# ax-le/nn-fac

Measured on NVIDIA B200. Metric: NMF outer iters/sec (HALS & MU beta=1) at 65536x8192 r=64, higher is better.
Workload: dtype f32

## Files before the change

include/nnfac_b200.h:

```cpp
#ifndef NNFAC_B200_H
#define NNFAC_B200_H

#include <stddef.h>
#include <stdint.h>

#ifdef __cplusplus
extern "C" {
#endif

#define NNFAC_ABI_VERSION 1

typedef enum { NNFAC_F32 = 0, NNFAC_F64 = 1 } nnfac_dtype;

typedef enum {
  NNFAC_OK = 0,
  NNFAC_ERR_ARG = -1,
  NNFAC_ERR_CUDA = -2,
  NNFAC_ERR_UNSUPPORTED = -3,
  NNFAC_ERR_ALLOC = -4
} nnfac_status;

#define NNFAC_HALS_NORMALIZE 1u
#define NNFAC_HALS_NONZERO 2u
#define NNFAC_HALS_NO_TC 4u

typedef struct nnfac_ctx nnfac_ctx;

int nnfac_abi_version(void);
const char* nnfac_last_error(void);
int nnfac_ctx_create(int device, nnfac_ctx** out);
int nnfac_ctx_destroy(nnfac_ctx* ctx);
int nnfac_ctx_sm_count(const nnfac_ctx* ctx);
int64_t nnfac_ctx_launch_count(const nnfac_ctx* ctx);

int nnfac_ctx_board_export(nnfac_ctx* ctx, void* handle_out);
int nnfac_ctx_board_attach(nnfac_ctx* ctx, int world, int rank, const void* handles);
int nnfac_ctx_collective(nnfac_ctx* ctx, int on, const int64_t* slice_lengths);
int nnfac_ctx_sweep_variant(nnfac_ctx* ctx, int mode);

typedef struct nnfac_xchg nnfac_xchg;
int nnfac_xchg_create(nnfac_ctx* ctx, int64_t stage_floats, int64_t send_floats, nnfac_xchg** out);
int nnfac_xchg_export(nnfac_xchg* x, void* handle_out);
int nnfac_xchg_attach(nnfac_xchg* x, int world, int rank, const void* handles);
int nnfac_xchg_destroy(nnfac_xchg* x);
void* nnfac_xchg_ptr(nnfac_xchg* x, int which);
int nnfac_xchg_post(nnfac_xchg* x, int phase, void* stream);
int nnfac_xchg_post_tail(nnfac_xchg* x, const float* tail_src, int rows, int64_t pitch, int64_t col, void* stream);
int nnfac_xchg_pull_tail(nnfac_xchg* x, int which, float* out, int64_t ld_out, int r, int64_t pitch, int64_t col, int tail, void* stream);
int nnfac_xchg_inbox_mu_apply(nnfac_xchg* x, int64_t inbox_off, int nslabs, int64_t slab_stride, int64_t chunk, int64_t tail_pitch,
                              const float* F, int64_t ld_f, int r, int64_t lo, int64_t ncols, double floor_value, int64_t ld_send,
                              void* stream);

int nnfac_hals_nnls(nnfac_ctx* ctx, int dtype, const void* UtM, int64_t ld_utm, const void* UtU,
                    int64_t ld_utu, void* V, int64_t ld_v, int r, int64_t n, int maxiter,
                    double delta, double sparsity, unsigned flags, double* result, void* stream);
int nnfac_hals_solve_f32(nnfac_ctx* ctx, const float* UtM, int64_t ld_utm, const float* UtU, int64_t ld_utu,
                         const float* Vin, int64_t ld_vin, float* Vout, int64_t ld_vout, int r, int64_t n, int maxiter,
                         double delta, double sparsity, double* result, void* stream);
int nnfac_hals_solve_slabs_f32(nnfac_ctx* ctx, const float* UtM, int64_t ld_utm, int nslabs, int64_t slab_stride, int r_pad,
                               float* scratch, const float* UtU, int64_t ld_utu, const float* Vin, int64_t ld_vin, float* Vout,
                               int64_t ld_vout, int r, int64_t n, int maxiter, double delta, double sparsity, double* result,
                               void* stream);

int nnfac_gemm_strided(nnfac_ctx* ctx, int dtype, void* C, int64_t ldc, int64_t sc_b, const void* A,
                       int64_t sa_i, int64_t sa_k, int64_t sa_q, int64_t sa_b, const void* B,
                       int64_t sb_k, int64_t sb_j, int64_t sb_q, int64_t sb_b, int64_t M, int64_t N,
                       int64_t K, int64_t kb, int64_t batch, void* stream);

int nnfac_gram(nnfac_ctx* ctx, int dtype, void* out, int64_t ld_out, const void* F, int64_t ld_f, int r,
               int64_t len, void* stream);

int nnfac_mu_terms(nnfac_ctx* ctx, int dtype, double beta, const void* K, const void* X, void* P,
                   void* Q, int64_t count, void* stream);

int nnfac_mu_apply(nnfac_ctx* ctx, int dtype, void* F_out, const void* F_in, const void* num,
                   const void* den_mat, const void* den_vec, int vec_per_row, int64_t rows,
                   int64_t cols, double gamma, double floor_value, void* stream);

int nnfac_beta_divergence(nnfac_ctx* ctx, int dtype, double beta, const void* A, const void* B,
                          int64_t count, double* out, void* stream);

int nnfac_sq_diff(nnfac_ctx* ctx, int dtype, const void* A, const void* B, int64_t count,
                  double* out, void* stream);

int nnfac_dot(nnfac_ctx* ctx, int dtype, const void* A, const void* B, int64_t count, double* out,
              void* stream);

int nnfac_row_sums(nnfac_ctx* ctx, int dtype, const void* A, int64_t lda, int64_t rows,
                   int64_t cols, void* out, void* stream);

int nnfac_norm1(nnfac_ctx* ctx, int dtype, const void* A, int64_t lda, int64_t rows, int64_t cols,
                double* out, void* stream);

int nnfac_transpose(nnfac_ctx* ctx, int dtype, void* out, int64_t ld_out, const void* in,
                    int64_t ld_in, int64_t rows, int64_t cols, void* stream);

int nnfac_khatri_rao(nnfac_ctx* ctx, int dtype, void* out, const void* A, int64_t I, const void* B,
                     int64_t J, int64_t r, void* stream);

int nnfac_hadamard(nnfac_ctx* ctx, int dtype, void* out, const void* A, const void* B,
                   int64_t count, void* stream);
int nnfac_axpby(nnfac_ctx* ctx, int dtype, void* out, double a, const void* X, double b, const void* Y, int64_t count,
                void* stream);

int nnfac_core_pg_step(nnfac_ctx* ctx, int dtype, void* core, const void* MtX, const void* P, int64_t count, double step,
                       double sparse, double delta, double* state, void* stream);
int nnfac_core_pg_step_dev(nnfac_ctx* ctx, int dtype, void* core, const void* MtX, const void* P, int64_t count, double delta,
                           double* state, void* stream);
int nnfac_core_pg_step3(nnfac_ctx* ctx, int dtype, void* core, const void* MtX, const void* M0, const void* M1, const void* M2,
                        int r0, int r1, int r2, void* Z, double step, double sparse, int dev_scalars, double delta, double* state,
                        void* stream);
int nnfac_normalize_rows(nnfac_ctx* ctx, int dtype, void* A, int64_t lda, int64_t rows,
                         int64_t cols, void* stream);

typedef struct nnfac_nmf_plan nnfac_nmf_plan;
int nnfac_nmf_plan_create(nnfac_ctx* ctx, int64_t m, int64_t n, int r, nnfac_nmf_plan** out);
int nnfac_nmf_plan_bytes(nnfac_ctx* ctx, int64_t m, int64_t n, int r, size_t* bytes);
int nnfac_nmf_plan_create_in(nnfac_ctx* ctx, int64_t m, int64_t n, int r, void* workspace, size_t workspace_bytes,
                             void* stream, nnfac_nmf_plan** out);
int nnfac_nmf_plan_bytes_sided(nnfac_ctx* ctx, int64_t m, int64_t n, int r, int sides, size_t* bytes);
int nnfac_nmf_plan_create_sided(nnfac_ctx* ctx, int64_t m, int64_t n, int r, int sides, void* workspace, size_t workspace_bytes,
                                void* stream, nnfac_nmf_plan** out);
int nnfac_nmf_plan_bytes_planes(nnfac_ctx* ctx, int64_t m, int64_t n, int r, int sides, int planes, size_t* bytes);
int nnfac_nmf_plan_create_planes(nnfac_ctx* ctx, int64_t m, int64_t n, int r, int sides, int planes, void* workspace,
                                 size_t workspace_bytes, void* stream, nnfac_nmf_plan** out);
int nnfac_nmf_plan_view_bytes(nnfac_ctx* ctx, const nnfac_nmf_plan* base, int64_t left, int64_t I, int64_t right, int r, size_t* bytes);
int nnfac_nmf_plan_create_view(nnfac_ctx* ctx, const nnfac_nmf_plan* base, int64_t left, int64_t I, int64_t right, int r,
                               void* workspace, size_t workspace_bytes, void* stream, nnfac_nmf_plan** out);
int nnfac_nmf_plan_destroy(nnfac_nmf_plan* plan);
int nnfac_nmf_plan_load_x(nnfac_nmf_plan* plan, const float* X, int64_t ldx, void* stream);
int nnfac_nmf_plan_load_x_rows(nnfac_nmf_plan* plan, const float* Xrows, int64_t ldx, int64_t row0, int64_t rows, void* stream);
int nnfac_nmf_plan_load_x_done(nnfac_nmf_plan* plan, void* stream);
int nnfac_nmf_plan_f32_bytes(const nnfac_nmf_plan* plan, size_t* bytes);
int nnfac_nmf_plan_enable_f32(nnfac_nmf_plan* plan, void* workspace, size_t workspace_bytes, void* stream);
int nnfac_nmf_plan_cross(nnfac_nmf_plan* plan, int which, const float* F, int64_t ldf, float* out,
                         int64_t ld_out, void* stream);
int nnfac_nmf_plan_set_krao(nnfac_nmf_plan* plan, const float* At, int64_t lda, int64_t I, const float* Bt, int64_t ldb,
                            int64_t J, void* stream);
int nnfac_nmf_plan_set_krao_rows(nnfac_nmf_plan* plan, const float* At, int64_t lda, int64_t I, const float* Bt, int64_t ldb,
                                 int64_t J, void* stream);
int nnfac_nmf_plan_reduce(nnfac_nmf_plan* plan, int side, float* out, int64_t ld_out, void* stream);
int nnfac_nmf_plan_reduce_chunked(nnfac_nmf_plan* plan, int side, float* out, int64_t chunk, int slabs, const float* tail,
                                  int64_t ld_tail, int tail_cols, void* stream);
int nnfac_nmf_plan_set_factor(nnfac_nmf_plan* plan, int which, const float* Ft, int64_t ld, void* stream);
int nnfac_nmf_plan_set_factor_gathered(nnfac_nmf_plan* plan, int which, const float* G, int64_t chunk, float* Ft_out,
                                       int64_t ld_out, void* stream);
int nnfac_nmf_plan_set_factor_pulled(nnfac_nmf_plan* plan, int which, const nnfac_xchg* x, int64_t chunk, int64_t pitch,
                                     float* Ft_out, int64_t ld_out, void* stream);
int nnfac_nmf_plan_set_push(nnfac_nmf_plan* plan, const nnfac_xchg* x, int64_t inbox_off, int64_t chunk, int* slabs,
                            int64_t* slab_stride);
int nnfac_reduce_slabs_f32(nnfac_ctx* ctx, const float* slabs, int64_t ld, int nslabs, int r, int r_pad, int64_t n, float* out,
                           int64_t ld_out, void* stream);
int nnfac_nmf_plan_hals_solve(nnfac_nmf_plan* plan, int which, const float* UtM, int64_t ld_utm, const float* UtU,
                              int64_t ld_utu, const float* F_in, int64_t ld_in, float* F_out, int64_t ld_out, int maxiter,
                              double delta, double sparsity, double* result, void* stream);
int nnfac_nmf_plan_fused(nnfac_nmf_plan* plan, int side, int mode, int want_cost, float* out, int64_t ld_out,
                         double* cost_out, void* stream);
int nnfac_nmf_plan_mu_finish(nnfac_nmf_plan* plan, int which, const float* F_in, int64_t ld_in, const float* den,
                             double floor_value, float* F_out, int64_t ld_out, void* stream);
int nnfac_nmf_plan_fused_beta_bytes(const nnfac_nmf_plan* plan, size_t* bytes);
int nnfac_nmf_plan_fused_beta(nnfac_nmf_plan* plan, int side, double beta, int want_cost, float* den_partial, double* cost_out,
                              void* stream);
int nnfac_nmf_plan_mu_finish_beta(nnfac_nmf_plan* plan, int which, const float* F_in, int64_t ld_in, const float* den_partial,
                                  double gamma, double floor_value, float* F_out, int64_t ld_out, void* stream);
int nnfac_nmf_plan_info(const nnfac_nmf_plan* plan, int which, int* splits, int* stages_per_unit,
                        int* num_units, int* num_stages, int* grid);

int nnfac_philox_uniform(nnfac_ctx* ctx, float* out, int64_t ld, int64_t rows, int64_t cols, int64_t row0, int64_t col0,
                         uint64_t seed, uint32_t stream_id, double scale, int accumulate, void* stream);

#ifdef __cplusplus
}
#endif
#endif
```

nn-fac_b200/csrc/tc_common.cuh:

```cuda
#pragma once
#include <cuda.h>
#include <cuda_bf16.h>
#include <stdint.h>

namespace tc {

__device__ __forceinline__ uint32_t smem_u32(const void* p) {
  return (uint32_t)__cvta_generic_to_shared(p);
}

__device__ __forceinline__ void mbar_init(uint64_t* bar, uint32_t count) {
  asm volatile("mbarrier.init.shared::cta.b64 [%0], %1;" ::"r"(smem_u32(bar)), "r"(count) : "memory");
}
__device__ __forceinline__ void fence_barrier_init() {
  asm volatile("fence.mbarrier_init.release.cluster;" ::: "memory");
}
__device__ __forceinline__ void mbar_arrive_expect_tx(uint64_t* bar, uint32_t bytes) {
  asm volatile("mbarrier.arrive.expect_tx.shared::cta.b64 _, [%0], %1;" ::"r"(smem_u32(bar)), "r"(bytes) : "memory");
}
__device__ __forceinline__ void mbar_arrive(uint64_t* bar) {
  asm volatile("mbarrier.arrive.shared::cta.b64 _, [%0];" ::"r"(smem_u32(bar)) : "memory");
}
__device__ __forceinline__ bool mbar_try_wait(uint64_t* bar, uint32_t parity) {
  uint32_t ok;
  asm volatile(
      "{\n"
      " .reg .pred p;\n"
      " mbarrier.try_wait.parity.shared::cta.b64 p, [%1], %2;\n"
      " selp.u32 %0, 1, 0, p;\n"
      "}\n"
      : "=r"(ok)
      : "r"(smem_u32(bar)), "r"(parity)
      : "memory");
  return ok != 0;
}
__device__ __forceinline__ uint64_t global_ns() {
  uint64_t t;
  asm volatile("mov.u64 %0, %globaltimer;" : "=l"(t));
  return t;
}
static __device__ __noinline__ void mbar_wait_timeout_check(uint64_t& t0) {
  const uint64_t now = global_ns();
  if (t0 == 0) t0 = now;
  else if (now - t0 > 4000000000ull) __trap();
}
__device__ __forceinline__ void mbar_wait(uint64_t* bar, uint32_t parity) {
  if (mbar_try_wait(bar, parity)) return;
  uint64_t t0 = 0;
  for (;;) {
#pragma unroll 1
    for (uint32_t spins = 0; spins < 4096u; ++spins)
      if (mbar_try_wait(bar, parity)) return;
    mbar_wait_timeout_check(t0);
  }
}

__device__ __forceinline__ void fence_proxy_async_smem() {
  asm volatile("fence.proxy.async.shared::cta;" ::: "memory");
}
__device__ __forceinline__ void tcgen05_fence_before() {
  asm volatile("tcgen05.fence::before_thread_sync;" ::: "memory");
}
__device__ __forceinline__ void tcgen05_fence_after() {
  asm volatile("tcgen05.fence::after_thread_sync;" ::: "memory");
}

__device__ __forceinline__ void prefetch_tmap(const CUtensorMap* m) {
  asm volatile("prefetch.tensormap [%0];" ::"l"(reinterpret_cast<uint64_t>(m)) : "memory");
}
__device__ __forceinline__ void tma_load_2d(void* smem_dst, const CUtensorMap* m, uint64_t* bar, int c0, int c1) {
  asm volatile(
      "cp.async.bulk.tensor.2d.shared::cluster.global.tile.mbarrier::complete_tx::bytes [%0], [%1, {%3, %4}], [%2];"
      ::"r"(smem_u32(smem_dst)), "l"(reinterpret_cast<uint64_t>(m)), "r"(smem_u32(bar)), "r"(c0), "r"(c1)
      : "memory");
}
__device__ __forceinline__ void tma_load_2d_hint(void* smem_dst, const CUtensorMap* m, uint64_t* bar, int c0, int c1,
                                                 uint64_t policy) {
  asm volatile(
      "cp.async.bulk.tensor.2d.shared::cluster.global.tile.mbarrier::complete_tx::bytes.L2::cache_hint [%0], [%1, {%3, %4}], [%2], %5;"
      ::"r"(smem_u32(smem_dst)), "l"(reinterpret_cast<uint64_t>(m)), "r"(smem_u32(bar)), "r"(c0), "r"(c1), "l"(policy)
      : "memory");
}
__device__ __forceinline__ void tma_load_3d_hint(void* smem_dst, const CUtensorMap* m, uint64_t* bar, int c0, int c1, int c2,
                                                 uint64_t policy) {
  asm volatile(
      "cp.async.bulk.tensor.3d.shared::cluster.global.tile.mbarrier::complete_tx::bytes.L2::cache_hint [%0], [%1, {%3, %4, %5}], [%2], %6;"
      ::"r"(smem_u32(smem_dst)), "l"(reinterpret_cast<uint64_t>(m)), "r"(smem_u32(bar)), "r"(c0), "r"(c1), "r"(c2), "l"(policy)
      : "memory");
}
constexpr uint64_t kEvictFirst = 0x12F0000000000000ull;
constexpr uint64_t kEvictLast = 0x14F0000000000000ull;

__device__ __forceinline__ void tmem_alloc(uint32_t* smem_result, uint32_t ncols) {
  asm volatile("tcgen05.alloc.cta_group::1.sync.aligned.shared::cta.b32 [%0], %1;" ::"r"(smem_u32(smem_result)), "r"(ncols)
               : "memory");
  asm volatile("tcgen05.relinquish_alloc_permit.cta_group::1.sync.aligned;" ::: "memory");
}
__device__ __forceinline__ void tmem_dealloc(uint32_t taddr, uint32_t ncols) {
  asm volatile("tcgen05.dealloc.cta_group::1.sync.aligned.b32 %0, %1;" ::"r"(taddr), "r"(ncols) : "memory");
}
__device__ __forceinline__ void tmem_ld16(uint32_t taddr, uint32_t (&v)[16]) {
  asm volatile(
      "tcgen05.ld.sync.aligned.32x32b.x16.b32 {%0,%1,%2,%3,%4,%5,%6,%7,%8,%9,%10,%11,%12,%13,%14,%15}, [%16];"
      : "=r"(v[0]), "=r"(v[1]), "=r"(v[2]), "=r"(v[3]), "=r"(v[4]), "=r"(v[5]), "=r"(v[6]), "=r"(v[7]), "=r"(v[8]),
        "=r"(v[9]), "=r"(v[10]), "=r"(v[11]), "=r"(v[12]), "=r"(v[13]), "=r"(v[14]), "=r"(v[15])
      : "r"(taddr)
      : "memory");
}
__device__ __forceinline__ void tmem_ld32(uint32_t taddr, uint32_t (&v)[32]) {
  asm volatile(
      "tcgen05.ld.sync.aligned.32x32b.x32.b32 {%0,%1,%2,%3,%4,%5,%6,%7,%8,%9,%10,%11,%12,%13,%14,%15,"
      "%16,%17,%18,%19,%20,%21,%22,%23,%24,%25,%26,%27,%28,%29,%30,%31}, [%32];"
      : "=r"(v[0]), "=r"(v[1]), "=r"(v[2]), "=r"(v[3]), "=r"(v[4]), "=r"(v[5]), "=r"(v[6]), "=r"(v[7]), "=r"(v[8]),
        "=r"(v[9]), "=r"(v[10]), "=r"(v[11]), "=r"(v[12]), "=r"(v[13]), "=r"(v[14]), "=r"(v[15]), "=r"(v[16]),
        "=r"(v[17]), "=r"(v[18]), "=r"(v[19]), "=r"(v[20]), "=r"(v[21]), "=r"(v[22]), "=r"(v[23]), "=r"(v[24]),
        "=r"(v[25]), "=r"(v[26]), "=r"(v[27]), "=r"(v[28]), "=r"(v[29]), "=r"(v[30]), "=r"(v[31])
      : "r"(taddr)
      : "memory");
}
__device__ __forceinline__ void tmem_st16(uint32_t taddr, const uint32_t (&v)[16]) {
  asm volatile(
      "tcgen05.st.sync.aligned.32x32b.x16.b32 [%0], {%1,%2,%3,%4,%5,%6,%7,%8,%9,%10,%11,%12,%13,%14,%15,%16};"
      ::"r"(taddr), "r"(v[0]), "r"(v[1]), "r"(v[2]), "r"(v[3]), "r"(v[4]), "r"(v[5]), "r"(v[6]), "r"(v[7]), "r"(v[8]),
        "r"(v[9]), "r"(v[10]), "r"(v[11]), "r"(v[12]), "r"(v[13]), "r"(v[14]), "r"(v[15])
      : "memory");
}
__device__ __forceinline__ void tmem_st8(uint32_t taddr, const uint32_t (&v)[8]) {
  asm volatile("tcgen05.st.sync.aligned.32x32b.x8.b32 [%0], {%1,%2,%3,%4,%5,%6,%7,%8};"
               ::"r"(taddr), "r"(v[0]), "r"(v[1]), "r"(v[2]), "r"(v[3]), "r"(v[4]), "r"(v[5]), "r"(v[6]), "r"(v[7])
               : "memory");
}
__device__ __forceinline__ void tmem_ld_wait16(uint32_t (&v)[16]) {
  asm volatile("tcgen05.wait::ld.sync.aligned;"
               : "+r"(v[0]), "+r"(v[1]), "+r"(v[2]), "+r"(v[3]), "+r"(v[4]), "+r"(v[5]), "+r"(v[6]), "+r"(v[7]), "+r"(v[8]),
                 "+r"(v[9]), "+r"(v[10]), "+r"(v[11]), "+r"(v[12]), "+r"(v[13]), "+r"(v[14]), "+r"(v[15])
               :
               : "memory");
}
__device__ __forceinline__ void tmem_st_wait() { asm volatile("tcgen05.wait::st.sync.aligned;" ::: "memory"); }
__device__ __forceinline__ void tmem_ld_wait() { asm volatile("tcgen05.wait::ld.sync.aligned;" ::: "memory"); }

__device__ __forceinline__ uint64_t umma_desc_k_sw128(uint32_t smem_addr) {
  uint64_t d = 0;
  d |= (uint64_t)((smem_addr >> 4) & 0x3FFF);
  d |= (uint64_t)1 << 16;
  d |= (uint64_t)(1024 >> 4) << 32;
  d |= (uint64_t)1 << 46;
  d |= (uint64_t)2 << 61;
  return d;
}
__device__ __forceinline__ uint64_t umma_desc_mn_sw128(uint32_t smem_addr) {
  uint64_t d = 0;
  d |= (uint64_t)((smem_addr >> 4) & 0x3FFF);
  d |= (uint64_t)(8192 >> 4) << 16;
  d |= (uint64_t)(1024 >> 4) << 32;
  d |= (uint64_t)1 << 46;
  d |= (uint64_t)2 << 61;
  return d;
}
__device__ __forceinline__ uint32_t umma_idesc_bf16(int M, int N) {
  return (1u << 4) | (1u << 7) | (1u << 10) | ((uint32_t)(N >> 3) << 17) | ((uint32_t)(M >> 4) << 24);
}
__device__ __forceinline__ void umma_bf16(uint32_t tmem_d, uint64_t adesc, uint64_t bdesc, uint32_t idesc, bool accumulate) {
  asm volatile(
      "{\n"
      " .reg .pred p;\n"
      " setp.ne.b32 p, %4, 0;\n"
      " tcgen05.mma.cta_group::1.kind::f16 [%0], %1, %2, %3, p;\n"
      "}\n" ::"r"(tmem_d), "l"(adesc), "l"(bdesc), "r"(idesc), "r"((uint32_t)accumulate)
      : "memory");
}
__device__ __forceinline__ void umma_bf16_ts(uint32_t tmem_d, uint32_t tmem_a, uint64_t bdesc, uint32_t idesc, bool accumulate) {
  asm volatile(
      "{\n"
      " .reg .pred p;\n"
      " setp.ne.b32 p, %4, 0;\n"
      " tcgen05.mma.cta_group::1.kind::f16 [%0], [%1], %2, %3, p;\n"
      "}\n" ::"r"(tmem_d), "r"(tmem_a), "l"(bdesc), "r"(idesc), "r"((uint32_t)accumulate)
      : "memory");
}
__device__ __forceinline__ void umma_commit(uint64_t* bar) {
  asm volatile("tcgen05.commit.cta_group::1.mbarrier::arrive::one.shared::cluster.b64 [%0];" ::"r"(smem_u32(bar)) : "memory");
}

__device__ __forceinline__ bool elect_one() {
  uint32_t pred;
  asm volatile(
      "{\n"
      " .reg .pred p;\n"
      " elect.sync _|p, 0xffffffff;\n"
      " selp.u32 %0, 1, 0, p;\n"
      "}\n"
      : "=r"(pred));
  return pred != 0;
}

__device__ __forceinline__ void split_bf16(float x, __nv_bfloat16& hi, __nv_bfloat16& lo) {
  hi = __float2bfloat16_rn(x);
  lo = __float2bfloat16_rn(x - __bfloat162float(hi));
}

__device__ __forceinline__ void split3_bf16(float x, __nv_bfloat16& hi, __nv_bfloat16& mid, __nv_bfloat16& lo) {
  hi = __float2bfloat16_rn(x);
  if (isinf(__bfloat162float(hi)) && isfinite(x)) hi = __float2bfloat16_rz(x);
  const float r = x - __bfloat162float(hi);
  mid = __float2bfloat16_rn(r);
  lo = __float2bfloat16_rn(r - __bfloat162float(mid));
}

}
```

nn-fac_b200/csrc/tc_fused.cu:

```cuda
#include "tc_plan.cuh"

#include <string.h>

namespace {
using namespace tcplan;

constexpr int NSP = 4;
constexpr int CW = 64 / NSP;
constexpr int NCHK = CW / 8;
constexpr int NWT = 4 * NSP;
constexpr int FUSED_THREADS = 128 + 32 * NWT;
static_assert(CW == 16, "the transform below moves 16 columns per tcgen05.ld / 8 words per tcgen05.st");
constexpr uint32_t X_BYTES = TILE_ROWS * BK * sizeof(bf16);
constexpr int MODE_RES = 0, MODE_MU = 1, MODE_BETA0 = 2, MODE_BETAI = 3, MODE_BETAG = 4;
#ifndef FUSED_PREFETCH
#define FUSED_PREFETCH 0
#endif
#ifndef FUSED_PACKED
#define FUSED_PACKED 1
#endif
#ifndef FUSED_DEFER_COST
#define FUSED_DEFER_COST 1
#endif
constexpr int DRAIN = 2;

template <int RK, int PLANES = 2, bool XF32 = false>
struct Cfg {
  static constexpr int KR = RK / 64;
  static constexpr uint32_t FK_BYTES = (uint32_t)KR * 64 * BK * sizeof(bf16);
  static constexpr uint32_t XB = (PLANES == 3 && !XF32 ? 3 : 2) * X_BYTES;
  static constexpr uint32_t STAGE_BYTES = XB + PLANES * FK_BYTES;
  static constexpr int FSTAGES = PLANES == 3 ? (XF32 ? 3 : 2) : RK == 64 ? 4 : 3;
  static constexpr int ND1 = PLANES == 3 && XF32 ? 2 : RK == 64 ? 3 : 2;
  static constexpr uint32_t A1_BYTES = RK == 64 ? PLANES * X_BYTES : 0;
  static constexpr int CWD = RK / NSP;
  static constexpr size_t SMEM = A1_BYTES + (size_t)FSTAGES * STAGE_BYTES + 512;
};

struct FusedParams {
  int r_pad, splits, stages_per_unit, num_units, drain, want_cost, tiles, split_major;
  int64_t ld_partial;
  float* partial;
  double* cost_part;
  const bf16 *a1h, *a1l;
  int64_t R;
  float* push[NNFAC_MAX_PEERS];
  int64_t push_chunk;
  int push_src;
};

constexpr int NHC = 11;
struct BetaParams {
  float* den;
  float beta, bm2;
  int ibm2, ibeta;
  float inv_bb1, inv_beta;
  float hc[NHC];
};

__device__ __forceinline__ float rcp_approx(float x) {
  float y;
  asm("rcp.approx.ftz.f32 %0, %1;" : "=f"(y) : "f"(x));
  return y;
}
__device__ __forceinline__ float lg2_approx(float x) {
  float y;
  asm("lg2.approx.ftz.f32 %0, %1;" : "=f"(y) : "f"(x));
  return y;
}
__device__ __forceinline__ float kl_g(float q) {
  const float d = q - 1.f;
  if (fabsf(d) < 0.0625f) {
    float c = fmaf(d, -1.f / 42.f, 1.f / 30.f);
    c = fmaf(d, c, -1.f / 20.f);
    c = fmaf(d, c, 1.f / 12.f);
    c = fmaf(d, c, -1.f / 6.f);
    c = fmaf(d, c, 0.5f);
    return d * d * c;
  }
  return fmaf(q, lg2_approx(q + 1e-30f) * 0.6931471805599453f, -d);
}
__device__ __forceinline__ float ex2_approx(float x) {
  float y;
  asm("ex2.approx.ftz.f32 %0, %1;" : "=f"(y) : "f"(x));
  return y;
}
__device__ __forceinline__ float ipow(float b, int n) {
  float r = 1.f;
  for (; n; n >>= 1, b *= b)
    if (n & 1) r *= b;
  return r;
}
template <int MODE>
__device__ __forceinline__ float beta_cost(float x, float k, float kb, float ik, const BetaParams& bp) {
  if (!(k > 0.f)) return 0.f;
  if (x == 0.f) return MODE == MODE_BETA0 ? -1.f : kb * bp.inv_beta;
  const float q = x * ik, d = q - 1.f;
  float h;
  if (fabsf(d) < 0.25f) {
    float c = bp.hc[NHC - 1];
#pragma unroll
    for (int i = NHC - 2; i >= 0; --i) c = fmaf(d, c, bp.hc[i]);
    h = d * d * c;
  } else if (MODE == MODE_BETA0) {
    h = fmaf(lg2_approx(q), -0.6931471805599453f, d);
  } else {
    const float qb = MODE == MODE_BETAI ? ipow(q, bp.ibeta) : ex2_approx(bp.beta * lg2_approx(q));
    h = (fmaf(-bp.beta, q, qb) + (bp.beta - 1.f)) * bp.inv_bb1;
  }
  return kb * h;
}
__device__ __forceinline__ float bf_lo(uint32_t w) { return __uint_as_float(w << 16); }
__device__ __forceinline__ float bf_hi(uint32_t w) { return __uint_as_float(w & 0xffff0000u); }

template <int MODE, bool COST, bool XF32, int RK, int PLANES = 2>
__global__ void __launch_bounds__(FUSED_THREADS, 1)
tc_fused_kernel(const __grid_constant__ CUtensorMap map_xh, const __grid_constant__ CUtensorMap map_xl,
                const __grid_constant__ CUtensorMap map_fkh, const __grid_constant__ CUtensorMap map_fkl,
                const __grid_constant__ CUtensorMap map_a1h, const __grid_constant__ CUtensorMap map_a1l,
                const FusedParams p, const __grid_constant__ CUtensorMap map_xm, const __grid_constant__ CUtensorMap map_fkm,
                const __grid_constant__ CUtensorMap map_a1m, const BetaParams bp) {
  using C = Cfg<RK, PLANES, PLANES == 3 && XF32>;
  constexpr bool BETA = MODE >= MODE_BETA0;
  static_assert(!BETA || (RK == 64 && PLANES == 2), "general beta: 2 planes, rank <= 64");
  static_assert(RK == 64 || (MODE == MODE_RES && !XF32), "rank 65..128: residual + cross-product pass only");
  static_assert(PLANES == 2 || (RK == 64 && (MODE == MODE_RES) != XF32), "3 planes: rank <= 64; beta = 1 reads X from its fp32 copy");
  constexpr int FSTAGES = C::FSTAGES, ND1 = BETA ? 2 : C::ND1, CWD = C::CWD;
  constexpr int NQ = BETA ? 1 : 2;
  constexpr int DRAIN_P = PLANES == 3 ? 1 : DRAIN;
  constexpr uint32_t FK_BYTES = C::FK_BYTES, STAGE_BYTES = C::STAGE_BYTES, A1_BYTES = C::A1_BYTES, XB = C::XB;
  extern __shared__ __align__(1024) uint8_t smem[];
  uint8_t* a1 = smem;
  uint8_t* ring = smem + A1_BYTES;
  uint64_t* bars = reinterpret_cast<uint64_t*>(ring + (size_t)FSTAGES * STAGE_BYTES);
  uint64_t* full = bars;
  uint64_t* empty = bars + 4;
  uint64_t* a1_full = bars + 9;
  uint64_t* a1_empty = bars + 10;
  uint64_t* d1_full = bars + 11;
  uint64_t* d1_empty = bars + 14;
  uint64_t* d2_full = bars + 17;
  uint64_t* d2_empty = bars + 19;
  uint64_t* a1t_ready = bars + 21;
  uint64_t* a1t_free = bars + 22;
  uint64_t* q_ready = bars + 23;
  uint64_t* q_free = bars + 25;
  uint32_t* tmem_slot = reinterpret_cast<uint32_t*>(bars + 27);
  double* cost_sh = reinterpret_cast<double*>(bars + 28);

  const int warp = threadIdx.x >> 5, lane = threadIdx.x & 31;

  if (warp == 0 && lane == 0) {
    tc::prefetch_tmap(&map_xh); tc::prefetch_tmap(&map_xl);
    tc::prefetch_tmap(&map_fkh); tc::prefetch_tmap(&map_fkl);
    if (RK == 64) { tc::prefetch_tmap(&map_a1h); tc::prefetch_tmap(&map_a1l); }
    if (PLANES == 3) { if (!XF32) tc::prefetch_tmap(&map_xm); tc::prefetch_tmap(&map_fkm); tc::prefetch_tmap(&map_a1m); }
  }
  if (warp == 1 && lane == 0) {
    for (int s = 0; s < FSTAGES; ++s) { tc::mbar_init(&full[s], 1); tc::mbar_init(&empty[s], NWT + 1); }
    tc::mbar_init(a1_full, 1); tc::mbar_init(a1_empty, BETA ? 1 : NWT);
    tc::mbar_init(a1t_ready, NWT); tc::mbar_init(a1t_free, 1);
    for (int b = 0; b < 2; ++b) { tc::mbar_init(&q_ready[b], NWT); tc::mbar_init(&q_free[b], 1); }
    for (int b = 0; b < ND1; ++b) { tc::mbar_init(&d1_full[b], 1); tc::mbar_init(&d1_empty[b], NWT); }
    for (int b = 0; b < 2; ++b) { tc::mbar_init(&d2_full[b], 1); tc::mbar_init(&d2_empty[b], NWT); }
    tc::fence_barrier_init();
  }
  if (warp == 2) tc::tmem_alloc(tmem_slot, 512);
  tc::tcgen05_fence_before();
  __syncthreads();
  tc::tcgen05_fence_after();
  const uint32_t tmem_base = *tmem_slot;
  const uint32_t D1 = tmem_base, D2 = tmem_base + 64 * ND1, A1T = D2 + 2 * RK, QT = BETA ? A1T + 2 * RK : A1T + PLANES * (RK / 2);
  const uint32_t D2D = A1T;
  const int S = p.stages_per_unit;

  if (warp == 0 && lane == 0) {
    int stage = 0; uint32_t phase = 0, a1_phase = 0;
    for (int u = blockIdx.x; u < p.num_units; u += gridDim.x) {
      const int tile = p.split_major ? u % p.tiles : u / p.splits, split = p.split_major ? u / p.tiles : u % p.splits;
      const int row0 = tile * TILE_ROWS, k0 = split * S * BK;
      if (RK == 64) {
        tc::mbar_wait(a1_empty, a1_phase ^ 1);
        a1_phase ^= 1;
        tc::mbar_arrive_expect_tx(a1_full, A1_BYTES);
        tc::tma_load_2d_hint(a1, &map_a1h, a1_full, 0, row0, tc::kEvictLast);
        tc::tma_load_2d_hint(a1 + X_BYTES, &map_a1l, a1_full, 0, row0, tc::kEvictLast);
        if (PLANES == 3) tc::tma_load_2d_hint(a1 + 2 * X_BYTES, &map_a1m, a1_full, 0, row0, tc::kEvictLast);
      }
      for (int ks = 0; ks < S; ++ks) {
        tc::mbar_wait(&empty[stage], phase ^ 1);
        uint8_t* st = ring + (size_t)stage * STAGE_BYTES;
        tc::mbar_arrive_expect_tx(&full[stage], STAGE_BYTES);
        const int c = k0 + ks * BK;
        tc::tma_load_2d_hint(st, &map_xh, &full[stage], c, row0, tc::kEvictFirst);
        tc::tma_load_2d_hint(st + X_BYTES, XF32 ? &map_xh : &map_xl, &full[stage], XF32 ? c + 32 : c, row0, tc::kEvictFirst);
        if (PLANES == 3 && !XF32) tc::tma_load_2d_hint(st + 2 * X_BYTES, &map_xm, &full[stage], c, row0, tc::kEvictFirst);
#pragma unroll
        for (int kr = 0; kr < C::KR; ++kr) {
          tc::tma_load_2d_hint(st + XB + kr * 8192, &map_fkh, &full[stage], kr * 64, c, tc::kEvictLast);
          tc::tma_load_2d_hint(st + XB + FK_BYTES + kr * 8192, &map_fkl, &full[stage], kr * 64, c, tc::kEvictLast);
          if (PLANES == 3) tc::tma_load_2d_hint(st + XB + 2 * FK_BYTES + kr * 8192, &map_fkm, &full[stage], kr * 64, c, tc::kEvictLast);
        }
        if (++stage == FSTAGES) { stage = 0; phase ^= 1; }
      }
    }
  } else if (warp == 1) {
    const uint32_t idesc1 = tc::umma_idesc_bf16(TILE_ROWS, 64);
    const int ksteps = p.r_pad / UMMA_K;
    int st1 = 0; uint32_t ph1 = 0;
    int b1 = 0; uint32_t b1_phase = 0;
    uint32_t a1_phase = 0;
    for (int u = blockIdx.x; u < p.num_units; u += gridDim.x) {
      tc::mbar_wait(BETA ? a1_full : a1t_ready, a1_phase);
      a1_phase ^= 1;
      for (int i = 0; i < S; ++i) {
        tc::mbar_wait(&full[st1], ph1);
        tc::mbar_wait(&d1_empty[b1], b1_phase ^ 1);
        tc::tcgen05_fence_after();
        if (tc::elect_one()) {
          const uint32_t sb = tc::smem_u32(ring + (size_t)st1 * STAGE_BYTES);
          const uint64_t fkh = tc::umma_desc_k_sw128(sb + XB), fkl = tc::umma_desc_k_sw128(sb + XB + FK_BYTES);
          const uint32_t d = D1 + (uint32_t)b1 * 64;
          if constexpr (PLANES == 3) {
            const uint64_t fkm = tc::umma_desc_k_sw128(sb + XB + 2 * FK_BYTES);
            const uint32_t ah = A1T, al = A1T + RK / 2, am = A1T + RK;
#pragma unroll
            for (int k = 0; k < RK / UMMA_K; ++k) {
              if (k < ksteps) {
                const uint64_t bo = (uint64_t)((k & 3) * 2);
                tc::umma_bf16_ts(d, al + 8 * k, fkh + bo, idesc1, k != 0);
                tc::umma_bf16_ts(d, am + 8 * k, fkm + bo, idesc1, true);
                tc::umma_bf16_ts(d, ah + 8 * k, fkl + bo, idesc1, true);
                tc::umma_bf16_ts(d, am + 8 * k, fkh + bo, idesc1, true);
                tc::umma_bf16_ts(d, ah + 8 * k, fkm + bo, idesc1, true);
              }
            }
#pragma unroll
            for (int k = 0; k < RK / UMMA_K; ++k)
              if (k < ksteps) tc::umma_bf16_ts(d, ah + 8 * k, fkh + (uint64_t)((k & 3) * 2), idesc1, true);
          } else if constexpr (BETA) {
            const uint64_t ah = tc::umma_desc_k_sw128(tc::smem_u32(a1)), al = tc::umma_desc_k_sw128(tc::smem_u32(a1 + X_BYTES));
#pragma unroll
            for (int k = 0; k < RK / UMMA_K; ++k) {
              if (k < ksteps) {
                const uint64_t ko = (uint64_t)(k * 2), bo = (uint64_t)((k & 3) * 2);
                tc::umma_bf16(d, ah + ko, fkh + bo, idesc1, k != 0);
                tc::umma_bf16(d, al + ko, fkh + bo, idesc1, true);
                tc::umma_bf16(d, ah + ko, fkl + bo, idesc1, true);
              }
            }
          } else {
#pragma unroll
          for (int k = 0; k < RK / UMMA_K; ++k) {
            if (k < ksteps) {
              const uint64_t bo = (uint64_t)((k >> 2) * (8192 >> 4) + (k & 3) * 2);
              tc::umma_bf16_ts(d, A1T + 8 * k, fkh + bo, idesc1, k != 0);
              tc::umma_bf16_ts(d, A1T + RK / 2 + 8 * k, fkh + bo, idesc1, true);
              tc::umma_bf16_ts(d, A1T + 8 * k, fkl + bo, idesc1, true);
            }
          }
          }
          tc::umma_commit(&d1_full[b1]);
          if (i == S - 1) tc::umma_commit(BETA ? a1_empty : a1t_free);
        }
        __syncwarp();
        if (++b1 == ND1) { b1 = 0; b1_phase ^= 1; }
        if (++st1 == FSTAGES) { st1 = 0; ph1 ^= 1; }
      }
    }
  } else if (warp == 3) {
    const uint32_t idesc2 = tc::umma_idesc_bf16(TILE_ROWS, p.r_pad) | (1u << 16);
    int qb = 0; uint32_t qb_phase = 0;
    int st2 = 0; uint32_t ph2 = 0;
    int b2 = 0; uint32_t b2_phase = 0;
    for (int u = blockIdx.x; u < p.num_units; u += gridDim.x) {
      for (int j = 0; j < S; ++j) {
        const bool chain_start = (j % DRAIN_P) == 0;
        const bool chain_end = ((j + 1) % DRAIN_P) == 0 || j == S - 1;
        tc::mbar_wait(&full[st2], ph2);
        if (MODE == MODE_MU || BETA) tc::mbar_wait(&q_ready[qb], qb_phase);
        if (chain_start) tc::mbar_wait(&d2_empty[b2], b2_phase ^ 1);
        tc::tcgen05_fence_after();
        if (tc::elect_one()) {
          const uint32_t sb = tc::smem_u32(ring + (size_t)st2 * STAGE_BYTES);
          const uint64_t xh = tc::umma_desc_k_sw128(sb), xl = tc::umma_desc_k_sw128(sb + X_BYTES);
          const uint64_t fnh = tc::umma_desc_mn_sw128(sb + XB);
          const uint64_t fnl = tc::umma_desc_mn_sw128(sb + XB + FK_BYTES);
          const uint32_t d = D2 + (uint32_t)b2 * RK;
          if constexpr (PLANES == 3) {
            const uint64_t fnm = tc::umma_desc_mn_sw128(sb + XB + 2 * FK_BYTES);
            const uint64_t xm = tc::umma_desc_k_sw128(sb + 2 * X_BYTES);
#pragma unroll
            for (int k = 0; k < BK / UMMA_K; ++k) {
              const uint64_t ko = (uint64_t)(k * 2), kb = (uint64_t)(k * 128);
              const bool acc0 = !(chain_start && k == 0);
              if (MODE == MODE_MU) {
                const uint32_t qa = QT + (uint32_t)qb * 64 + 8 * k;
                tc::umma_bf16_ts(d, qa, fnl + kb, idesc2, acc0);
                tc::umma_bf16_ts(d, qa + 32, fnm + kb, idesc2, true);
                tc::umma_bf16_ts(d, qa, fnm + kb, idesc2, true);
                tc::umma_bf16_ts(d, qa + 32, fnh + kb, idesc2, true);
              } else {
                tc::umma_bf16(d, xl + ko, fnh + kb, idesc2, acc0);
                tc::umma_bf16(d, xm + ko, fnm + kb, idesc2, true);
                tc::umma_bf16(d, xh + ko, fnl + kb, idesc2, true);
                tc::umma_bf16(d, xm + ko, fnh + kb, idesc2, true);
                tc::umma_bf16(d, xh + ko, fnm + kb, idesc2, true);
              }
            }
#pragma unroll
            for (int k = 0; k < BK / UMMA_K; ++k) {
              if (MODE == MODE_MU) tc::umma_bf16_ts(d, QT + (uint32_t)qb * 64 + 8 * k, fnh + (uint64_t)(k * 128), idesc2, true);
              else tc::umma_bf16(d, xh + (uint64_t)(k * 2), fnh + (uint64_t)(k * 128), idesc2, true);
            }
          } else if constexpr (BETA) {
            const uint32_t dd = D2D + (uint32_t)b2 * RK;
#pragma unroll
            for (int k = 0; k < BK / UMMA_K; ++k) {
              const uint64_t kb = (uint64_t)(k * 128);
              const uint32_t qa = QT + 8 * k, qd = qa + 64;
              const bool acc0 = !(chain_start && k == 0);
              tc::umma_bf16_ts(d, qa, fnh + kb, idesc2, acc0);
              tc::umma_bf16_ts(d, qa + 32, fnh + kb, idesc2, true);
              tc::umma_bf16_ts(d, qa, fnl + kb, idesc2, true);
              tc::umma_bf16_ts(dd, qd, fnh + kb, idesc2, acc0);
              tc::umma_bf16_ts(dd, qd + 32, fnh + kb, idesc2, true);
              tc::umma_bf16_ts(dd, qd, fnl + kb, idesc2, true);
            }
          } else {
#pragma unroll
          for (int k = 0; k < BK / UMMA_K; ++k) {
            const uint64_t ko = (uint64_t)(k * 2);
            const uint64_t kb = (uint64_t)(k * 128);
            if (MODE == MODE_MU) {
              const uint32_t qa = QT + (uint32_t)qb * 64 + 8 * k;
              tc::umma_bf16_ts(d, qa, fnh + kb, idesc2, !(chain_start && k == 0));
              tc::umma_bf16_ts(d, qa + 32, fnh + kb, idesc2, true);
              tc::umma_bf16_ts(d, qa, fnl + kb, idesc2, true);
            } else {
              tc::umma_bf16(d, xh + ko, fnh + kb, idesc2, !(chain_start && k == 0));
              tc::umma_bf16(d, xl + ko, fnh + kb, idesc2, true);
              tc::umma_bf16(d, xh + ko, fnl + kb, idesc2, true);
            }
          }
          }
          tc::umma_commit(&empty[st2]);
          if (MODE == MODE_MU || BETA) tc::umma_commit(&q_free[qb]);
          if (chain_end) tc::umma_commit(&d2_full[b2]);
        }
        __syncwarp();
        if (MODE == MODE_MU || BETA) { if (++qb == NQ) { qb = 0; qb_phase ^= 1; } }
        if (chain_end) { if (++b2 == 2) { b2 = 0; b2_phase ^= 1; } }
        if (++st2 == FSTAGES) { st2 = 0; ph2 ^= 1; }
      }
    }
  } else if (warp >= 4) {
    const int q = warp & 3, part = (warp - 4) >> 2;
    const int row = q * 32 + lane;
    const uint32_t lane_base = (uint32_t)(q * 32) << 16;
    int st = 0; uint32_t ph = 0;
    int b1 = 0; uint32_t b1_phase = 0;
    int b2 = 0; uint32_t b2_phase = 0;
    int qb = 0; uint32_t qb_phase = 0;
    uint32_t a1_phase = 0;
    double cost = 0.0, costk = 0.0;
    for (int u = blockIdx.x; u < p.num_units; u += gridDim.x) {
      const int tile = p.split_major ? u % p.tiles : u / p.splits, split = p.split_major ? u / p.tiles : u % p.splits;
      float sum[CWD], sumd[BETA ? CWD : 1];
#pragma unroll
      for (int j = 0; j < CWD; ++j) sum[j] = 0.f;
      if (BETA) {
#pragma unroll
        for (int j = 0; j < CWD; ++j) sumd[BETA ? j : 0] = 0.f;
      } else if (RK == 64) {
        tc::mbar_wait(a1_full, a1_phase);
        tc::mbar_wait(a1t_free, a1_phase ^ 1);
        a1_phase ^= 1;
        tc::tcgen05_fence_after();
#pragma unroll
        for (int pl = 0; pl < PLANES; ++pl) {
          uint32_t w[4 * NCHK];
#pragma unroll
          for (int cc = 0; cc < NCHK; ++cc) {
            const int chunk = NCHK * part + cc;
            const uint4 v4 = *reinterpret_cast<const uint4*>(a1 + pl * X_BYTES + (uint32_t)row * 128u + (uint32_t)((chunk ^ (row & 7)) << 4));
            w[4 * cc] = v4.x; w[4 * cc + 1] = v4.y; w[4 * cc + 2] = v4.z; w[4 * cc + 3] = v4.w;
          }
          tc::tmem_st8(A1T + lane_base + 32 * pl + (CW / 2) * part, w);
        }
        tc::tmem_st_wait();
        tc::tcgen05_fence_before();
        __syncwarp();
        if (lane == 0) { tc::mbar_arrive(a1t_ready); tc::mbar_arrive(a1_empty); }
      } else {
        const int64_t grow = (int64_t)tile * TILE_ROWS + row;
        uint32_t w[2][16];
#pragma unroll
        for (int pl = 0; pl < 2; ++pl) {
          const uint4* src = reinterpret_cast<const uint4*>((pl ? p.a1l : p.a1h) + grow * RK + part * (RK / 4));
#pragma unroll
          for (int c = 0; c < 4; ++c) {
            const uint4 v4 = grow < p.R ? __ldg(src + c) : make_uint4(0u, 0u, 0u, 0u);
            w[pl][4 * c] = v4.x; w[pl][4 * c + 1] = v4.y; w[pl][4 * c + 2] = v4.z; w[pl][4 * c + 3] = v4.w;
          }
        }
        tc::mbar_wait(a1t_free, a1_phase ^ 1);
        a1_phase ^= 1;
        tc::tcgen05_fence_after();
        tc::tmem_st16(A1T + lane_base + (RK / 8) * part, w[0]);
        tc::tmem_st16(A1T + lane_base + RK / 2 + (RK / 8) * part, w[1]);
        tc::tmem_st_wait();
        tc::tcgen05_fence_before();
        __syncwarp();
        if (lane == 0) tc::mbar_arrive(a1t_ready);
      }
      auto drain_chain = [&]() {
        tc::mbar_wait(&d2_full[b2], b2_phase);
        tc::tcgen05_fence_after();
#pragma unroll
        for (int c0 = 0; c0 < CWD; c0 += 16) {
          if (CWD * part + c0 < p.r_pad) {
            uint32_t v[16];
            tc::tmem_ld16(D2 + (uint32_t)b2 * RK + lane_base + CWD * part + c0, v);
            tc::tmem_ld_wait();
#pragma unroll
            for (int j = 0; j < 16; ++j) sum[c0 + j] += __uint_as_float(v[j]);
            if (BETA) {
              tc::tmem_ld16(D2D + (uint32_t)b2 * RK + lane_base + CWD * part + c0, v);
              tc::tmem_ld_wait();
#pragma unroll
              for (int j = 0; j < 16; ++j) sumd[BETA ? c0 + j : 0] += __uint_as_float(v[j]);
            }
          }
        }
        tc::tcgen05_fence_before();
        __syncwarp();
        if (lane == 0) tc::mbar_arrive(&d2_empty[b2]);
        if (++b2 == 2) { b2 = 0; b2_phase ^= 1; }
      };
      int drained = 0;
      float2 acc2 = make_float2(0.f, 0.f), acck2 = make_float2(0.f, 0.f);
      const float2 neg1 = make_float2(-1.f, -1.f), tiny2 = make_float2(1e-30f, 1e-30f);
      uint32_t kn[CW];
      int bf = b1; uint32_t bf_phase = b1_phase;
      auto fetch_d1 = [&]() {
        tc::mbar_wait(&d1_full[bf], bf_phase);
        tc::tcgen05_fence_after();
        tc::tmem_ld16(D1 + (uint32_t)bf * 64 + lane_base + CW * part, kn);
        if (++bf == ND1) { bf = 0; bf_phase ^= 1; }
      };
#if FUSED_PREFETCH
      fetch_d1();
#endif
      for (int i = 0; i < S; ++i) {
#if !FUSED_PREFETCH
        fetch_d1();
#endif
        tc::tmem_ld_wait16(kn);
        uint32_t kk[CW];
#pragma unroll
        for (int j = 0; j < CW; ++j) kk[j] = kn[j];
        tc::tcgen05_fence_before();
        __syncwarp();
        if (lane == 0) tc::mbar_arrive(&d1_empty[b1]);
        if (++b1 == ND1) { b1 = 0; b1_phase ^= 1; }
#if FUSED_PREFETCH
        if (i + 1 < S) fetch_d1();
#endif
        tc::mbar_wait(&full[st], ph);
        uint8_t* xh = ring + (size_t)st * STAGE_BYTES;
        uint8_t* xl = xh + X_BYTES;
        uint32_t qhw[4 * NCHK], qlw[4 * NCHK];
        constexpr bool DEFER = FUSED_DEFER_COST && FUSED_PACKED && MODE == MODE_MU && COST;
        float2 xs[DEFER ? 4 * NCHK : 1], qs[DEFER ? 4 * NCHK : 1];
        uint32_t dhw[BETA ? 4 * NCHK : 1], dlw[BETA ? 4 * NCHK : 1];
#pragma unroll
        for (int cc = 0; cc < NCHK; ++cc) {
          float2 xv[4];
          if (XF32) {
            const uint8_t* xb = xh + (size_t)(part >> 1) * X_BYTES + (uint32_t)row * 128u;
#pragma unroll
            for (int h = 0; h < 2; ++h) {
              const int chunk = 4 * (part & 1) + 2 * cc + h;
              const float4 v4 = *reinterpret_cast<const float4*>(xb + ((chunk ^ (row & 7)) << 4));
              xv[2 * h] = make_float2(v4.x, v4.y); xv[2 * h + 1] = make_float2(v4.z, v4.w);
            }
          } else {
            const int chunk = NCHK * part + cc;
            const uint32_t off = (uint32_t)row * 128u + (uint32_t)((chunk ^ (row & 7)) << 4);
            const uint4 h4 = *reinterpret_cast<const uint4*>(xh + off);
            const uint4 l4 = *reinterpret_cast<const uint4*>(xl + off);
            const uint32_t hw[4] = {h4.x, h4.y, h4.z, h4.w}, lw[4] = {l4.x, l4.y, l4.z, l4.w};
            if constexpr (PLANES == 3) {
              const uint4 m4 = *reinterpret_cast<const uint4*>(xl + X_BYTES + off);
              const uint32_t mw[4] = {m4.x, m4.y, m4.z, m4.w};
#pragma unroll
              for (int w = 0; w < 4; ++w)
                xv[w] = __fadd2_rn(make_float2(bf_lo(hw[w]), bf_hi(hw[w])),
                                   __fadd2_rn(make_float2(bf_lo(mw[w]), bf_hi(mw[w])), make_float2(bf_lo(lw[w]), bf_hi(lw[w]))));
            } else {
#pragma unroll
            for (int w = 0; w < 4; ++w)
#if FUSED_PACKED
              xv[w] = __fadd2_rn(make_float2(bf_lo(hw[w]), bf_hi(hw[w])), make_float2(bf_lo(lw[w]), bf_hi(lw[w])));
#else
              xv[w] = make_float2(bf_lo(hw[w]) + bf_lo(lw[w]), bf_hi(hw[w]) + bf_hi(lw[w]));
#endif
            }
          }
          if constexpr (BETA) {
#pragma unroll
            for (int w = 0; w < 4; ++w) {
              float an[2], ad[2];
#pragma unroll
              for (int h = 0; h < 2; ++h) {
                const float x = h ? xv[w].y : xv[w].x, k = __uint_as_float(kk[cc * 8 + 2 * w + h]);
                float ik = 0.f, pk, kb = 1.f;
                if (MODE == MODE_BETA0) {
                  ik = rcp_approx(k);
                  pk = ik * ik;
                  ad[h] = ik;
                } else {
                  pk = MODE == MODE_BETAI ? ipow(k, bp.ibm2) : ex2_approx(bp.bm2 * lg2_approx(k));
                  ad[h] = pk * k;
                  if (COST) { ik = rcp_approx(k); kb = ad[h] * k; }
                }
                an[h] = x * pk;
                if (!(k > 0.f)) { an[h] = 0.f; ad[h] = 0.f; }
                if (COST) acc2.x += beta_cost<MODE>(x, k, kb, ik, bp);
              }
              const __nv_bfloat162 hn = __floats2bfloat162_rn(an[0], an[1]), hd = __floats2bfloat162_rn(ad[0], ad[1]);
              const uint32_t hnw = *reinterpret_cast<const uint32_t*>(&hn), hdw = *reinterpret_cast<const uint32_t*>(&hd);
              const __nv_bfloat162 ln = __floats2bfloat162_rn(an[0] - bf_lo(hnw), an[1] - bf_hi(hnw));
              const __nv_bfloat162 ld = __floats2bfloat162_rn(ad[0] - bf_lo(hdw), ad[1] - bf_hi(hdw));
              qhw[4 * cc + w] = hnw;
              qlw[4 * cc + w] = *reinterpret_cast<const uint32_t*>(&ln);
              dhw[BETA ? 4 * cc + w : 0] = hdw;
              dlw[BETA ? 4 * cc + w : 0] = *reinterpret_cast<const uint32_t*>(&ld);
            }
          } else {
#if FUSED_PACKED
#pragma unroll
          for (int w = 0; w < 4; ++w) {
            const float2 x2 = xv[w];
            const float2 k2 = make_float2(__uint_as_float(kk[cc * 8 + 2 * w]), __uint_as_float(kk[cc * 8 + 2 * w + 1]));
            if (MODE == MODE_RES) {
              const float2 r2 = __ffma2_rn(k2, neg1, x2);
              acc2 = __ffma2_rn(r2, r2, acc2);
            } else {
              const float2 kt = __fadd2_rn(k2, tiny2);
              const float2 q2 = __fmul2_rn(x2, make_float2(rcp_approx(kt.x), rcp_approx(kt.y)));
              if (COST) {
                if (DEFER) {
                  xs[DEFER ? 4 * cc + w : 0] = x2; qs[DEFER ? 4 * cc + w : 0] = q2;
                } else {
                  const float2 qt = __fadd2_rn(q2, tiny2);
                  acc2 = __ffma2_rn(x2, make_float2(lg2_approx(qt.x), lg2_approx(qt.y)), acc2);
                }
                acck2 = __fadd2_rn(acck2, k2);
              }
              const __nv_bfloat162 hq = __floats2bfloat162_rn(q2.x, q2.y);
              const uint32_t hqw = *reinterpret_cast<const uint32_t*>(&hq);
              const float2 rem = __ffma2_rn(make_float2(bf_lo(hqw), bf_hi(hqw)), neg1, q2);
              const __nv_bfloat162 lq = __floats2bfloat162_rn(rem.x, rem.y);
              qhw[4 * cc + w] = hqw;
              qlw[4 * cc + w] = *reinterpret_cast<const uint32_t*>(&lq);
            }
          }
#else
#pragma unroll
          for (int w = 0; w < 4; ++w) {
            const float x0 = xv[w].x, x1 = xv[w].y;
            const float k0 = __uint_as_float(kk[cc * 8 + 2 * w]), k1 = __uint_as_float(kk[cc * 8 + 2 * w + 1]);
            if (MODE == MODE_RES) {
              const float r0 = x0 - k0, r1 = x1 - k1;
              acc2.x = fmaf(r0, r0, acc2.x);
              acc2.y = fmaf(r1, r1, acc2.y);
            } else {
              const float i0 = rcp_approx(fmaxf(k0, 1e-30f)), i1 = rcp_approx(fmaxf(k1, 1e-30f));
              const float q0 = x0 * i0, q1 = x1 * i1;
              if (COST) {
                acc2.x = fmaf(x0, lg2_approx(fmaxf(q0, 1e-30f)), acc2.x);
                acc2.y = fmaf(x1, lg2_approx(fmaxf(q1, 1e-30f)), acc2.y);
                acck2.x += k0; acck2.y += k1;
              }
              const __nv_bfloat162 hq = __floats2bfloat162_rn(q0, q1);
              const uint32_t hqw = *reinterpret_cast<const uint32_t*>(&hq);
              const __nv_bfloat162 lq = __floats2bfloat162_rn(q0 - bf_lo(hqw), q1 - bf_hi(hqw));
              qhw[4 * cc + w] = hqw;
              qlw[4 * cc + w] = *reinterpret_cast<const uint32_t*>(&lq);
            }
          }
#endif
          }
        }
        auto flush_cost = [&]() {
          if (COST && ((i & 7) == 7 || i == S - 1)) {
            cost += (double)(acc2.x + acc2.y);
            acc2 = make_float2(0.f, 0.f);
            if (MODE == MODE_MU) { costk += (double)(acck2.x + acck2.y); acck2 = make_float2(0.f, 0.f); }
          }
        };
        if (!DEFER) flush_cost();
        __syncwarp();
        if (lane == 0) tc::mbar_arrive(&empty[st]);
        if (++st == FSTAGES) { st = 0; ph ^= 1; }
        if (MODE == MODE_MU) {
          tc::mbar_wait(&q_free[qb], qb_phase ^ 1);
          tc::tcgen05_fence_after();
          const uint32_t qa = QT + (uint32_t)qb * 64 + lane_base + (CW / 2) * part;
          tc::tmem_st8(qa, qhw);
          tc::tmem_st8(qa + 32, qlw);
          tc::tmem_st_wait();
          tc::tcgen05_fence_before();
          __syncwarp();
          if (lane == 0) tc::mbar_arrive(&q_ready[qb]);
          if (++qb == NQ) { qb = 0; qb_phase ^= 1; }
          if (DEFER) {
#pragma unroll
            for (int e = 0; e < 4 * NCHK; ++e) {
              if constexpr (PLANES == 3) {
                const float2 k2 = make_float2(__uint_as_float(kk[2 * e]), __uint_as_float(kk[2 * e + 1]));
                acc2 = __ffma2_rn(k2, make_float2(kl_g(qs[DEFER ? e : 0].x), kl_g(qs[DEFER ? e : 0].y)), acc2);
              } else {
                const float2 qt = __fadd2_rn(qs[DEFER ? e : 0], tiny2);
                acc2 = __ffma2_rn(xs[DEFER ? e : 0], make_float2(lg2_approx(qt.x), lg2_approx(qt.y)), acc2);
              }
            }
            flush_cost();
          }
        }
        if constexpr (BETA) {
          tc::mbar_wait(&q_free[0], qb_phase ^ 1);
          tc::tcgen05_fence_after();
          const uint32_t qa = QT + lane_base + (CW / 2) * part;
          tc::tmem_st8(qa, qhw);
          tc::tmem_st8(qa + 32, qlw);
          tc::tmem_st8(qa + 64, dhw);
          tc::tmem_st8(qa + 96, dlw);
          tc::tmem_st_wait();
          tc::tcgen05_fence_before();
          __syncwarp();
          if (lane == 0) tc::mbar_arrive(&q_ready[0]);
          qb_phase ^= 1;
        }
        if (DRAIN_P == 2 ? (i >= 3 && (i & 1)) : i >= 2) { drain_chain(); ++drained; }
      }
      for (; drained < (S + DRAIN_P - 1) / DRAIN_P; ++drained) drain_chain();
      if (p.push_chunk > 0) {
        const int64_t row0 = (int64_t)tile * TILE_ROWS;
        const int q = (int)(row0 / p.push_chunk);
        float* out = p.push[q] + (((int64_t)p.push_src * p.splits + split) * p.r_pad + CWD * part) * p.push_chunk + (row0 - q * p.push_chunk) + row;
#pragma unroll
        for (int j = 0; j < CWD; ++j)
          if (CWD * part + j < p.r_pad) out[(int64_t)j * p.push_chunk] = sum[j];
      } else {
        float* out = p.partial + ((int64_t)split * p.r_pad + CWD * part) * p.ld_partial + (int64_t)tile * TILE_ROWS + row;
#pragma unroll
        for (int j = 0; j < CWD; ++j)
          if (CWD * part + j < p.r_pad) out[(int64_t)j * p.ld_partial] = sum[j];
        if (BETA) {
          float* outd = bp.den + ((int64_t)split * p.r_pad + CWD * part) * p.ld_partial + (int64_t)tile * TILE_ROWS + row;
#pragma unroll
          for (int j = 0; j < CWD; ++j)
            if (CWD * part + j < p.r_pad) outd[(int64_t)j * p.ld_partial] = sumd[BETA ? j : 0];
        }
      }
    }
    if (COST) {
      cost = warp_sum(cost);
      if (MODE == MODE_MU) costk = warp_sum(costk);
      if (lane == 0) { cost_sh[warp - 4] = cost; cost_sh[NWT + warp - 4] = costk; }
      asm volatile("bar.sync 1, %0;" ::"n"(32 * NWT) : "memory");
      if (warp == 4 && lane == 0) {
        double t = 0.0, tk = 0.0;
        for (int w = 0; w < NWT; ++w) { t += cost_sh[w]; tk += cost_sh[NWT + w]; }
        p.cost_part[blockIdx.x] = t;
        p.cost_part[512 + blockIdx.x] = tk;
      }
    }
  }
  tc::tcgen05_fence_before();
  __syncthreads();
  if (warp == 2) tc::tmem_dealloc(tmem_base, 512);
}

struct PeerG {
  const float* p[NNFAC_MAX_PEERS];
  const unsigned long long* flags;
  int world;
  unsigned long long seq;
};

template <bool APPLY, int RK, bool PULL, int PLANES = 2, bool DENP = false>
__global__ void __launch_bounds__(256) factor_finish_kernel(const float* __restrict__ partial, int splits, int r, int r_pad, int64_t R,
                                                            int64_t ldp, const float* __restrict__ F_in, int64_t ld_in,
                                                            int64_t in_chunk, int64_t in_slab, const PeerG G,
                                                            const float* __restrict__ den, float floor_value, float* __restrict__ F_out,
                                                            int64_t ld_out, bf16* __restrict__ fh, bf16* __restrict__ fl, int64_t ld_plane,
                                                            bf16* __restrict__ rowh, bf16* __restrict__ rowl,
                                                            bf16* __restrict__ fm = nullptr, bf16* __restrict__ rowm = nullptr,
                                                            float gamma = 1.f) {
  __shared__ float tile[RK][33];
  const int tx = threadIdx.x & 31, ty = threadIdx.x >> 5;
  if (PULL && G.flags != nullptr) {
    if ((int)threadIdx.x < G.world) {
      const unsigned long long* f = G.flags + NNFAC_MAX_PEERS + threadIdx.x;
      unsigned long long v, spins = 0;
      do {
        asm volatile("ld.acquire.sys.global.u64 %0, [%1];" : "=l"(v) : "l"(f) : "memory");
        if (++spins > (1ull << 27)) __trap();
      } while (v < G.seq);
    }
    __syncthreads();
  }
  const int64_t c0 = (int64_t)blockIdx.x * 32, c = c0 + tx;
  const int64_t cin = in_chunk > 0 ? (c / in_chunk) * in_slab + (c % in_chunk) : c;
  float pulled[PULL ? RK / 8 : 1];
  if (PULL) {
    const float* src = c < R ? G.p[c / in_chunk] + (c % in_chunk) : nullptr;
#pragma unroll
    for (int i = 0; i < RK / 8; ++i) {
      const int k = ty + 8 * i;
      pulled[i] = (k < r && c < R) ? __ldcv(src + (int64_t)k * ld_in) : 0.f;
    }
  }
#pragma unroll
  for (int k = ty; k < RK; k += 8) {
    float f = 0.f;
    if (k < r && c < R) {
      f = PULL ? pulled[PULL ? (k - ty) / 8 : 0] : F_in[(int64_t)k * ld_in + cin];
      if (APPLY) {
        auto sum_splits = [&](const float* __restrict__ part) {
          float s = 0.f;
          int sp = 0;
          for (; sp + 8 <= splits; sp += 8) {
            float t[8];
#pragma unroll
            for (int u = 0; u < 8; ++u) t[u] = part[((int64_t)(sp + u) * r_pad + k) * ldp + c];
#pragma unroll
            for (int u = 0; u < 8; ++u) s += t[u];
          }
          for (; sp < splits; ++sp) s += part[((int64_t)sp * r_pad + k) * ldp + c];
          return s;
        };
        const float num = sum_splits(partial);
        float v;
        if constexpr (DENP) {
          float ratio = num / sum_splits(den);
          if (gamma == 0.5f) ratio = sqrtf(ratio);
          else if (gamma != 1.f) ratio = powf(ratio, gamma);
          v = f * ratio;
        } else {
          v = f * (num / den[k]);
        }
        f = v > floor_value ? v : floor_value;
        if (v != v) f = v;
      }
      if (F_out) F_out[(int64_t)k * ld_out + c] = f;
      bf16 h, l;
      if constexpr (PLANES == 3) {
        bf16 md;
        tc::split3_bf16(f, h, md, l);
        fm[(int64_t)k * ld_plane + c] = md;
      } else {
        tc::split_bf16(f, h, l);
      }
      fh[(int64_t)k * ld_plane + c] = h;
      fl[(int64_t)k * ld_plane + c] = l;
    }
    tile[k][tx] = f;
  }
  if (rowh == nullptr) return;
  __syncthreads();
  for (int i = ty; i < 32; i += 8) {
    const int64_t cc = c0 + i;
    if (cc < R) {
#pragma unroll
      for (int h2 = 0; h2 < RK / 32; ++h2) {
        const int k = tx + 32 * h2;
        bf16 h, l;
        if constexpr (PLANES == 3) {
          bf16 md;
          tc::split3_bf16(tile[k][i], h, md, l);
          rowm[cc * RK + k] = md;
        } else {
          tc::split_bf16(tile[k][i], h, l);
        }
        rowh[cc * RK + k] = h;
        rowl[cc * RK + k] = l;
      }
    }
  }
}

__global__ void sum_cost_parts_kernel(const double* part, int n, double* out) {
  if (threadIdx.x == 0) {
    double s = 0.0;
    for (int i = 0; i < n; ++i) s += part[i];
    out[0] = s;
  }
}

__global__ void kl_cost_finish_kernel(const double* part, int n, const double* sums, double* out) {
  if (threadIdx.x == 0) {
    double s = 0.0, sk = 0.0;
    for (int i = 0; i < n; ++i) { s += part[i]; sk += part[512 + i]; }
    constexpr double a0 = 6.05e-8, a1 = -4.0e-8;
    s = (1.0 - a1) * s - a0 * sums[0];
    out[0] = 0.6931471805599453 * s - sums[0] + sk;
  }
}

template <int PLANES>
__global__ void __launch_bounds__(256) planes_to_f32_kernel(const bf16* __restrict__ hi, const bf16* __restrict__ lo, int64_t count,
                                                            float* __restrict__ out, const bf16* __restrict__ mid) {
  const int64_t stride = (int64_t)gridDim.x * blockDim.x * 2;
  for (int64_t i = ((int64_t)blockIdx.x * blockDim.x + threadIdx.x) * 2; i < count; i += stride) {
    const uint32_t h = *reinterpret_cast<const uint32_t*>(hi + i), l = *reinterpret_cast<const uint32_t*>(lo + i);
    if constexpr (PLANES == 3) {
      const uint32_t md = *reinterpret_cast<const uint32_t*>(mid + i);
      *reinterpret_cast<float2*>(out + i) = make_float2(bf_lo(h) + (bf_lo(md) + bf_lo(l)), bf_hi(h) + (bf_hi(md) + bf_hi(l)));
    } else {
      *reinterpret_cast<float2*>(out + i) = make_float2(bf_lo(h) + bf_lo(l), bf_hi(h) + bf_hi(l));
    }
  }
}

}

static int finish_factor(nnfac_nmf_plan* p, int which, bool apply, const float* F_in, int64_t ld_in, int64_t in_chunk, int64_t in_slab,
                         const float* den, float floor_value, float* F_out, int64_t ld_out, cudaStream_t st, const PeerG* pulled = nullptr) {
  const int64_t len = which == 0 ? p->m : p->n;
  Side* cs = &p->side[which == 0 ? 1 : 0];
  Side* ps = &p->side[which];
  const unsigned grid = (unsigned)ceil_div64(len, 32);
  bf16* rh = p->fused_ok ? p->rowp_h[which] : nullptr;
  bf16* rl = p->fused_ok ? p->rowp_l[which] : nullptr;
  PeerG none;
  memset(&none, 0, sizeof(none));
  if (p->planes == 3) {
    factor_finish_kernel<false, 64, false, 3><<<grid, 256, 0, st>>>(nullptr, 0, p->r, p->r_pad, len, 0, F_in, ld_in, in_chunk, in_slab,
        none, nullptr, 0.f, F_out, ld_out, cs->fh, cs->fl, cs->ld, rh, rl, cs->fm, p->rowp_m[which]);
    NNFAC_LAUNCH_CHECK(p->ctx);
    return NNFAC_OK;
  }
#define NNFAC_FINISH(RKV)                                                                                                          \
  do {                                                                                                                             \
    if (pulled)                                                                                                                    \
      factor_finish_kernel<false, RKV, true><<<grid, 256, 0, st>>>(nullptr, 0, p->r, p->r_pad, len, 0, nullptr, ld_in, in_chunk,  \
          in_slab, *pulled, nullptr, 0.f, F_out, ld_out, cs->fh, cs->fl, cs->ld, rh, rl);                                          \
    else if (apply)                                                                                                                \
      factor_finish_kernel<true, RKV, false><<<grid, 256, 0, st>>>(p->partial, ps->cp.splits, p->r, p->r_pad, len,                \
          ps->cp.ld_partial, F_in, ld_in, in_chunk, in_slab, none, den, floor_value, F_out, ld_out, cs->fh, cs->fl, cs->ld, rh,    \
          rl);                                                                                                                     \
    else                                                                                                                           \
      factor_finish_kernel<false, RKV, false><<<grid, 256, 0, st>>>(nullptr, 0, p->r, p->r_pad, len, 0, F_in, ld_in, in_chunk,    \
          in_slab, none, nullptr, 0.f, F_out, ld_out, cs->fh, cs->fl, cs->ld, rh, rl);                                             \
  } while (0)
  if (p->rk == 64) NNFAC_FINISH(64); else NNFAC_FINISH(128);
#undef NNFAC_FINISH
  NNFAC_LAUNCH_CHECK(p->ctx);
  return NNFAC_OK;
}

static FusedParams fused_params(const nnfac_nmf_plan* p, int side, bool want_cost) {
  const Side* s = &p->side[side];
  FusedParams fp;
  fp.r_pad = p->r_pad; fp.splits = s->cp.splits; fp.stages_per_unit = s->cp.stages_per_unit; fp.num_units = s->cp.num_units;
  fp.drain = DRAIN; fp.want_cost = want_cost ? 1 : 0;
  fp.tiles = s->cp.tiles; fp.split_major = s->cp.split_major;
  fp.ld_partial = s->cp.ld_partial; fp.partial = p->partial; fp.cost_part = p->cost_part;
  fp.a1h = p->rowp_h[side]; fp.a1l = p->rowp_l[side]; fp.R = s->R;
  fp.push_chunk = 0; fp.push_src = 0;
  for (int q = 0; q < NNFAC_MAX_PEERS; ++q) fp.push[q] = nullptr;
  return fp;
}

extern "C" {

int nnfac_nmf_plan_f32_bytes(const nnfac_nmf_plan* p, size_t* bytes) {
  NNFAC_ARG(p && bytes, "nnfac_nmf_plan_f32_bytes: NULL argument");
  size_t tot = 0;
  for (int i = 0; i < 2; ++i) tot += (((size_t)p->side[i].R * p->side[i].ld * sizeof(float)) + 255) & ~(size_t)255;
  *bytes = tot;
  return NNFAC_OK;
}

int nnfac_nmf_plan_enable_f32(nnfac_nmf_plan* p, void* workspace, size_t workspace_bytes, void* stream) {
  NNFAC_ARG(p && workspace && (((uintptr_t)workspace) & 255) == 0, "nnfac_nmf_plan_enable_f32: bad argument");
  size_t need = 0;
  nnfac_nmf_plan_f32_bytes(p, &need);
  NNFAC_ARG(workspace_bytes >= need, "nnfac_nmf_plan_enable_f32: workspace of %zu bytes needed, got %zu", need, workspace_bytes);
  NNFAC_ARG(p->sides == 3, "nnfac_nmf_plan_enable_f32: needs a two-sided plan");
  if (!p->fused_ok || p->rk != 64) { nnfac_set_error("nnfac_nmf_plan_enable_f32: rank %d > 64 is not covered by the beta = 1 fused pass", p->r); return NNFAC_ERR_UNSUPPORTED; }
  cudaStream_t st = (cudaStream_t)stream;
  uint8_t* base = (uint8_t*)workspace;
  for (int i = 0; i < 2; ++i) {
    Side* s = &p->side[i];
    p->xf[i] = (float*)base;
    const int64_t count = s->R * s->ld;
    base += (((size_t)count * sizeof(float)) + 255) & ~(size_t)255;
    if (p->planes == 3) planes_to_f32_kernel<3><<<p->ctx->sm_count * 16, 256, 0, st>>>(s->xh, s->xl, count, p->xf[i], s->xm);
    else planes_to_f32_kernel<2><<<p->ctx->sm_count * 16, 256, 0, st>>>(s->xh, s->xl, count, p->xf[i], nullptr);
    NNFAC_LAUNCH_CHECK(p->ctx);
    const int rc = make_map_f32(&p->map_xf[i], p->xf[i], s->R, s->C, s->ld);
    if (rc) return rc;
  }
  p->xf_ready = 1;
  return NNFAC_OK;
}

int nnfac_nmf_plan_set_factor(nnfac_nmf_plan* p, int which, const float* Ft, int64_t ld, void* stream) {
  NNFAC_ARG(p && Ft && (which == 0 || which == 1), "nnfac_nmf_plan_set_factor: bad argument");
  NNFAC_ARG(!p->base, "nnfac_nmf_plan_set_factor: not available on a view plan");
  const int64_t len = which == 0 ? p->m : p->n;
  NNFAC_ARG(ld >= len, "nnfac_nmf_plan_set_factor: leading dimension too small");
  return finish_factor(p, which, false, Ft, ld, 0, 0, nullptr, 0.f, nullptr, 0, (cudaStream_t)stream);
}

int nnfac_nmf_plan_set_factor_gathered(nnfac_nmf_plan* p, int which, const float* G, int64_t chunk, float* Ft_out, int64_t ld_out,
                                       void* stream) {
  NNFAC_ARG(p && G && Ft_out && chunk > 0 && (which == 0 || which == 1), "nnfac_nmf_plan_set_factor_gathered: bad argument");
  const int64_t len = which == 0 ? p->m : p->n;
  NNFAC_ARG(ld_out >= len, "nnfac_nmf_plan_set_factor_gathered: leading dimension too small");
  if (p->planes != 2) { nnfac_set_error("nnfac_nmf_plan_set_factor_gathered: writes two planes, the plan has %d", p->planes); return NNFAC_ERR_UNSUPPORTED; }
  return finish_factor(p, which, false, G, chunk, chunk, (int64_t)p->r * chunk, nullptr, 0.f, Ft_out, ld_out, (cudaStream_t)stream);
}

const float* nnfac_xchg_peer_send(const nnfac_xchg* x, int q);
int nnfac_xchg_world(const nnfac_xchg* x);
void nnfac_xchg_wait_args(const nnfac_xchg* x, int phase, const unsigned long long** flags, int* world, unsigned long long* seq);
int nnfac_nmf_plan_set_factor_pulled(nnfac_nmf_plan* p, int which, const nnfac_xchg* x, int64_t chunk, int64_t pitch, float* Ft_out,
                                     int64_t ld_out, void* stream) {
  NNFAC_ARG(p && x && Ft_out && chunk > 0 && pitch >= chunk && (which == 0 || which == 1), "nnfac_nmf_plan_set_factor_pulled: bad argument");
  NNFAC_ARG(!p->base, "nnfac_nmf_plan_set_factor_pulled: not available on a view plan");
  if (p->planes != 2) { nnfac_set_error("nnfac_nmf_plan_set_factor_pulled: writes two planes, the plan has %d", p->planes); return NNFAC_ERR_UNSUPPORTED; }
  const int64_t len = which == 0 ? p->m : p->n;
  const int world = nnfac_xchg_world(x);
  NNFAC_ARG(ld_out >= len && (int64_t)world * chunk >= len, "nnfac_nmf_plan_set_factor_pulled: %d slices of %lld columns do not cover %lld",
            world, (long long)chunk, (long long)len);
  PeerG g;
  for (int q = 0; q < NNFAC_MAX_PEERS; ++q) g.p[q] = nnfac_xchg_peer_send(x, q);
  nnfac_xchg_wait_args(x, 1, &g.flags, &g.world, &g.seq);
  return finish_factor(p, which, false, nullptr, pitch, chunk, 0, nullptr, 0.f, Ft_out, ld_out, (cudaStream_t)stream, &g);
}

int nnfac_nmf_plan_hals_solve(nnfac_nmf_plan* p, int which, const float* UtM, int64_t ld_utm, const float* UtU, int64_t ld_utu,
                              const float* F_in, int64_t ld_in, float* F_out, int64_t ld_out, int maxiter, double delta,
                              double sparsity, double* result, void* stream) {
  NNFAC_ARG(p && UtU && F_in && F_out && result && (which == 0 || which == 1), "nnfac_nmf_plan_hals_solve: bad argument");
  NNFAC_ARG(!p->base, "nnfac_nmf_plan_hals_solve: not available on a view plan");
  if (p->planes != 2) return NNFAC_ERR_UNSUPPORTED;
  const int64_t len = which == 0 ? p->m : p->n;
  NNFAC_ARG((!UtM || ld_utm >= len) && ld_in >= len && ld_out >= len && ld_utu >= p->r, "nnfac_nmf_plan_hals_solve: leading dimension too small");
  int nsplit = 1;
  int64_t split_stride = 0;
  if (!UtM) {
    const CrossParams& cp = p->side[which].cp;
    UtM = p->partial; ld_utm = cp.ld_partial; nsplit = cp.splits; split_stride = (int64_t)p->r_pad * cp.ld_partial;
  }
  Side* cs = &p->side[which == 0 ? 1 : 0];
  nnfac_sweep_planes pl;
  pl.fh = cs->fh; pl.fl = cs->fl; pl.ld_plane = cs->ld; pl.r_pad = p->r_pad;
  pl.rowh = p->fused_ok ? p->rowp_h[which] : nullptr;
  pl.rowl = p->fused_ok ? p->rowp_l[which] : nullptr;
  pl.row_pitch = p->rk;
  return nnfac_tc_sweep_run(p->ctx, UtM, ld_utm, UtU, ld_utu, F_in, ld_in, F_out, ld_out, p->r, len, maxiter, delta, sparsity,
                            result, &pl, (cudaStream_t)stream, nsplit, split_stride);
}

void* nnfac_xchg_peer_stage(const nnfac_xchg* x, int q);
int nnfac_xchg_rank(const nnfac_xchg* x);
int64_t nnfac_xchg_stage_floats(const nnfac_xchg* x);
int nnfac_nmf_plan_set_push(nnfac_nmf_plan* p, const nnfac_xchg* x, int64_t inbox_off, int64_t chunk, int* slabs, int64_t* slab_stride) {
  NNFAC_ARG(p, "nnfac_nmf_plan_set_push: NULL plan");
  if (!x) { p->push_chunk = 0; return NNFAC_OK; }
  NNFAC_ARG(!p->base && p->fused_ok, "nnfac_nmf_plan_set_push: needs a plan with the fused pass");
  if (p->planes != 2) { nnfac_set_error("nnfac_nmf_plan_set_push: not available on a 3-plane plan"); return NNFAC_ERR_UNSUPPORTED; }
  const int world = nnfac_xchg_world(x);
  const int splits = p->side[0].cp.splits;
  NNFAC_ARG(chunk > 0 && chunk % TILE_ROWS == 0 && (int64_t)world * chunk >= p->m && inbox_off >= 0,
            "nnfac_nmf_plan_set_push: %d slices of %lld rows (multiple of 128) must cover %lld", world, (long long)chunk, (long long)p->m);
  NNFAC_ARG(inbox_off + (int64_t)world * splits * p->r_pad * chunk <= nnfac_xchg_stage_floats(x),
            "nnfac_nmf_plan_set_push: the stage buffer is too small for %d x %d slabs of %d x %lld", world, splits, p->r_pad, (long long)chunk);
  for (int q = 0; q < world; ++q) p->push[q] = (float*)nnfac_xchg_peer_stage(x, q) + inbox_off;
  p->push_chunk = chunk; p->push_src = nnfac_xchg_rank(x); p->push_world = world;
  if (slabs) *slabs = world * splits;
  if (slab_stride) *slab_stride = (int64_t)p->r_pad * chunk;
  return NNFAC_OK;
}

int nnfac_reduce_slabs_f32(nnfac_ctx* ctx, const float* slabs, int64_t ld, int nslabs, int r, int r_pad, int64_t n, float* out,
                           int64_t ld_out, void* stream) {
  NNFAC_ARG(ctx && slabs && out && nslabs >= 1 && r >= 1 && r_pad >= r && n >= 1 && ld >= n && ld_out >= n, "nnfac_reduce_slabs_f32: bad argument");
  nnfac_reduce_partials(slabs, nslabs, r, r_pad, n, ld, out, ld_out, ctx->sm_count, (cudaStream_t)stream);
  NNFAC_LAUNCH_CHECK(ctx);
  return NNFAC_OK;
}

int nnfac_nmf_plan_reduce(nnfac_nmf_plan* p, int side, float* out, int64_t ld_out, void* stream) {
  NNFAC_ARG(p && out && (side == 0 || side == 1), "nnfac_nmf_plan_reduce: bad argument");
  Side* s = &p->side[side];
  NNFAC_ARG(ld_out >= s->R, "nnfac_nmf_plan_reduce: leading dimension too small");
  nnfac_reduce_partials(p->partial, s->cp.splits, p->r, p->r_pad, s->R, s->cp.ld_partial, out, ld_out, p->ctx->sm_count, (cudaStream_t)stream);
  NNFAC_LAUNCH_CHECK(p->ctx);
  return NNFAC_OK;
}

int nnfac_nmf_plan_reduce_chunked(nnfac_nmf_plan* p, int side, float* out, int64_t chunk, int slabs, const float* tail, int64_t ld_tail,
                                  int tail_cols, void* stream) {
  NNFAC_ARG(p && out && (side == 0 || side == 1) && chunk > 0 && slabs > 0 && tail_cols >= 0 && (tail || tail_cols == 0),
            "nnfac_nmf_plan_reduce_chunked: bad argument");
  Side* s = &p->side[side];
  NNFAC_ARG((int64_t)slabs * chunk >= s->R, "nnfac_nmf_plan_reduce_chunked: %d slabs of %lld columns do not cover %lld", slabs,
            (long long)chunk, (long long)s->R);
  nnfac_reduce_partials_chunked(p->partial, s->cp.splits, p->r, p->r_pad, s->R, s->cp.ld_partial, out, chunk, slabs, tail, ld_tail,
                                tail_cols, p->ctx->sm_count, (cudaStream_t)stream);
  NNFAC_LAUNCH_CHECK(p->ctx);
  return NNFAC_OK;
}

int nnfac_nmf_plan_mu_finish(nnfac_nmf_plan* p, int which, const float* F_in, int64_t ld_in, const float* den, double floor_value,
                             float* F_out, int64_t ld_out, void* stream) {
  NNFAC_ARG(p && F_in && den && F_out && (which == 0 || which == 1), "nnfac_nmf_plan_mu_finish: bad argument");
  const int64_t len = which == 0 ? p->m : p->n;
  NNFAC_ARG(ld_in >= len && ld_out >= len, "nnfac_nmf_plan_mu_finish: leading dimension too small");
  if (!p->fused_ok) { nnfac_set_error("nnfac_nmf_plan_mu_finish: rank %d > 128 is not covered by the fused pass", p->r); return NNFAC_ERR_UNSUPPORTED; }
  if (p->planes != 2) { nnfac_set_error("nnfac_nmf_plan_mu_finish: writes two planes, the plan has %d (apply + set_factor)", p->planes); return NNFAC_ERR_UNSUPPORTED; }
  return finish_factor(p, which, true, F_in, ld_in, 0, 0, den, (float)floor_value, F_out, ld_out, (cudaStream_t)stream);
}

int nnfac_nmf_plan_fused(nnfac_nmf_plan* p, int side, int mode, int want_cost, float* out, int64_t ld_out, double* cost_out,
                         void* stream) {
  NNFAC_ARG(p && (side == 0 || side == 1) && (mode == 0 || mode == 1), "nnfac_nmf_plan_fused: bad argument");
  NNFAC_ARG((p->sides >> side) & 1, "nnfac_nmf_plan_fused: this plan keeps no planes of side %d", side);
  if (!p->fused_ok) { nnfac_set_error("nnfac_nmf_plan_fused: not covered by the fused pass (rank %d > 128, or a view plan)", p->r); return NNFAC_ERR_UNSUPPORTED; }
  if (mode == 1 && p->rk != 64) { nnfac_set_error("nnfac_nmf_plan_fused: the beta = 1 pass covers rank <= 64 (rank %d)", p->r); return NNFAC_ERR_UNSUPPORTED; }
  if (mode == 1 && p->planes == 3 && !p->xf_ready) { nnfac_set_error("nnfac_nmf_plan_fused: the beta = 1 pass of a 3-plane plan reads X from its fp32 copies (nnfac_nmf_plan_enable_f32)"); return NNFAC_ERR_UNSUPPORTED; }
  Side* s = &p->side[side];
  NNFAC_ARG(!out || ld_out >= s->R, "nnfac_nmf_plan_fused: leading dimension too small");
  cudaStream_t st = (cudaStream_t)stream;
  FusedParams fp = fused_params(p, side, mode == 0 || want_cost);
  BetaParams bp;
  memset(&bp, 0, sizeof(bp));
  if (side == 0 && !out && p->push_chunk > 0) {
    fp.push_chunk = p->push_chunk; fp.push_src = p->push_src;
    for (int q = 0; q < p->push_world; ++q) fp.push[q] = p->push[q];
  }
  const int other = 1 - side;
#define NNFAC_LAUNCH_FUSED(M, C, XF, RKV, MAPH, MAPL)                                                                             \
  do {                                                                                                                        \
    const size_t smem = Cfg<RKV>::SMEM;                                                                                       \
    NNFAC_CUDA(cudaFuncSetAttribute(tc_fused_kernel<M, C, XF, RKV>, cudaFuncAttributeMaxDynamicSharedMemorySize, (int)smem)); \
    tc_fused_kernel<M, C, XF, RKV><<<s->grid, FUSED_THREADS, smem, st>>>(MAPH, MAPL, p->map_row_b_h[other],                  \
        p->map_row_b_l[other], p->map_row_a_h[side], p->map_row_a_l[side], fp, MAPH, p->map_row_b_h[other],                  \
        p->map_row_a_h[side], bp);                                                                                            \
  } while (0)
#define NNFAC_LAUNCH_FUSED3(M, C, XF, MAPH, MAPL)                                                                                \
  do {                                                                                                                        \
    const size_t smem = Cfg<64, 3, XF>::SMEM;                                                                                 \
    NNFAC_CUDA(cudaFuncSetAttribute(tc_fused_kernel<M, C, XF, 64, 3>, cudaFuncAttributeMaxDynamicSharedMemorySize, (int)smem)); \
    tc_fused_kernel<M, C, XF, 64, 3><<<s->grid, FUSED_THREADS, smem, st>>>(MAPH, MAPL, p->map_row_b_h[other],                \
        p->map_row_b_l[other], p->map_row_a_h[side], p->map_row_a_l[side], fp, s->map_xm, p->map_row_b_m[other],             \
        p->map_row_a_m[side], bp);                                                                                            \
  } while (0)
  if (p->planes == 3) {
    if (mode == 0) NNFAC_LAUNCH_FUSED3(MODE_RES, true, false, s->map_xh, s->map_xl);
    else if (fp.want_cost) NNFAC_LAUNCH_FUSED3(MODE_MU, true, true, p->map_xf[side], p->map_xf[side]);
    else NNFAC_LAUNCH_FUSED3(MODE_MU, false, true, p->map_xf[side], p->map_xf[side]);
  } else if (mode == 0 && p->rk == 128) NNFAC_LAUNCH_FUSED(MODE_RES, true, false, 128, s->map_xh, s->map_xl);
  else if (mode == 0) NNFAC_LAUNCH_FUSED(MODE_RES, true, false, 64, s->map_xh, s->map_xl);
  else if (p->xf_ready) {
    if (fp.want_cost) NNFAC_LAUNCH_FUSED(MODE_MU, true, true, 64, p->map_xf[side], p->map_xf[side]);
    else NNFAC_LAUNCH_FUSED(MODE_MU, false, true, 64, p->map_xf[side], p->map_xf[side]);
  } else {
    if (fp.want_cost) NNFAC_LAUNCH_FUSED(MODE_MU, true, false, 64, s->map_xh, s->map_xl);
    else NNFAC_LAUNCH_FUSED(MODE_MU, false, false, 64, s->map_xh, s->map_xl);
  }
#undef NNFAC_LAUNCH_FUSED
#undef NNFAC_LAUNCH_FUSED3
  NNFAC_LAUNCH_CHECK(p->ctx);
  if (out) {
    nnfac_reduce_partials(p->partial, fp.splits, p->r, p->r_pad, s->R, fp.ld_partial, out, ld_out, p->ctx->sm_count, st);
    NNFAC_LAUNCH_CHECK(p->ctx);
  }
  if (cost_out && fp.want_cost) {
    if (mode == 0 || p->planes == 3)
      sum_cost_parts_kernel<<<1, 32, 0, st>>>(p->cost_part, s->grid, cost_out);
    else
      kl_cost_finish_kernel<<<1, 32, 0, st>>>(p->cost_part, s->grid, p->sums, cost_out);
    NNFAC_LAUNCH_CHECK(p->ctx);
  }
  return NNFAC_OK;
}

int nnfac_nmf_plan_fused_beta_bytes(const nnfac_nmf_plan* p, size_t* bytes) {
  NNFAC_ARG(p && bytes, "nnfac_nmf_plan_fused_beta_bytes: NULL argument");
  *bytes = p->partial_bytes;
  return NNFAC_OK;
}

int nnfac_nmf_plan_fused_beta(nnfac_nmf_plan* p, int side, double beta, int want_cost, float* den_partial, double* cost_out,
                              void* stream) {
  NNFAC_ARG(p && den_partial && (side == 0 || side == 1), "nnfac_nmf_plan_fused_beta: bad argument");
  NNFAC_ARG(beta >= 0.0, "nnfac_nmf_plan_fused_beta: beta must be >= 0 (got %g)", beta);
  NNFAC_ARG((p->sides >> side) & 1, "nnfac_nmf_plan_fused_beta: this plan keeps no planes of side %d", side);
  if (beta == 1.0 || beta == 2.0) { nnfac_set_error("nnfac_nmf_plan_fused_beta: beta = %g is the mode-1 / cross-product pass", beta); return NNFAC_ERR_UNSUPPORTED; }
  if (p->base) { nnfac_set_error("nnfac_nmf_plan_fused_beta: not available on a view plan"); return NNFAC_ERR_UNSUPPORTED; }
  if (!p->fused_ok || p->rk != 64) { nnfac_set_error("nnfac_nmf_plan_fused_beta: covers rank <= 64 (rank %d)", p->r); return NNFAC_ERR_UNSUPPORTED; }
  if (p->planes != 2) { nnfac_set_error("nnfac_nmf_plan_fused_beta: covers 2-plane plans (the plan has %d)", p->planes); return NNFAC_ERR_UNSUPPORTED; }
  if (p->push_chunk > 0) { nnfac_set_error("nnfac_nmf_plan_fused_beta: not available with the push exchange (nnfac_nmf_plan_set_push)"); return NNFAC_ERR_UNSUPPORTED; }
  Side* s = &p->side[side];
  cudaStream_t st = (cudaStream_t)stream;
  const FusedParams fp = fused_params(p, side, want_cost != 0);
  BetaParams bp;
  memset(&bp, 0, sizeof(bp));
  bp.den = den_partial;
  bp.beta = (float)beta; bp.bm2 = (float)(beta - 2.0);
  bp.ibm2 = (int)beta - 2; bp.ibeta = (int)beta;
  bp.inv_bb1 = (float)(1.0 / (beta * (beta - 1.0))); bp.inv_beta = beta > 0.0 ? (float)(1.0 / beta) : 0.f;
  double c = 0.5;
  for (int i = 0; i < NHC; ++i) { bp.hc[i] = (float)c; c *= (beta - (i + 2)) / (i + 3); }
  const bool integral = beta >= 3.0 && beta == (double)(int)beta;
  const int other = 1 - side;
#define NNFAC_LAUNCH_BETA(M, C, XF, MAPH, MAPL)                                                                                \
  do {                                                                                                                        \
    const size_t smem = Cfg<64>::SMEM;                                                                                        \
    NNFAC_CUDA(cudaFuncSetAttribute(tc_fused_kernel<M, C, XF, 64>, cudaFuncAttributeMaxDynamicSharedMemorySize, (int)smem));  \
    tc_fused_kernel<M, C, XF, 64><<<s->grid, FUSED_THREADS, smem, st>>>(MAPH, MAPL, p->map_row_b_h[other],                    \
        p->map_row_b_l[other], p->map_row_a_h[side], p->map_row_a_l[side], fp, MAPH, p->map_row_b_h[other],                  \
        p->map_row_a_h[side], bp);                                                                                            \
  } while (0)
#define NNFAC_LAUNCH_BETA_X(M, C)                                                                                              \
  do {                                                                                                                        \
    if (p->xf_ready) NNFAC_LAUNCH_BETA(M, C, true, p->map_xf[side], p->map_xf[side]);                                         \
    else NNFAC_LAUNCH_BETA(M, C, false, s->map_xh, s->map_xl);                                                                \
  } while (0)
  if (beta == 0.0) { if (fp.want_cost) NNFAC_LAUNCH_BETA_X(MODE_BETA0, true); else NNFAC_LAUNCH_BETA_X(MODE_BETA0, false); }
  else if (integral) { if (fp.want_cost) NNFAC_LAUNCH_BETA_X(MODE_BETAI, true); else NNFAC_LAUNCH_BETA_X(MODE_BETAI, false); }
  else { if (fp.want_cost) NNFAC_LAUNCH_BETA_X(MODE_BETAG, true); else NNFAC_LAUNCH_BETA_X(MODE_BETAG, false); }
#undef NNFAC_LAUNCH_BETA_X
#undef NNFAC_LAUNCH_BETA
  NNFAC_LAUNCH_CHECK(p->ctx);
  if (cost_out && fp.want_cost) {
    sum_cost_parts_kernel<<<1, 32, 0, st>>>(p->cost_part, s->grid, cost_out);
    NNFAC_LAUNCH_CHECK(p->ctx);
  }
  return NNFAC_OK;
}

int nnfac_nmf_plan_mu_finish_beta(nnfac_nmf_plan* p, int which, const float* F_in, int64_t ld_in, const float* den_partial, double gamma,
                                  double floor_value, float* F_out, int64_t ld_out, void* stream) {
  NNFAC_ARG(p && F_in && den_partial && F_out && (which == 0 || which == 1), "nnfac_nmf_plan_mu_finish_beta: bad argument");
  const int64_t len = which == 0 ? p->m : p->n;
  NNFAC_ARG(ld_in >= len && ld_out >= len, "nnfac_nmf_plan_mu_finish_beta: leading dimension too small");
  if (p->base || !p->fused_ok || p->rk != 64 || p->planes != 2) {
    nnfac_set_error("nnfac_nmf_plan_mu_finish_beta: covers the plans of nnfac_nmf_plan_fused_beta (rank <= 64, 2 planes, no view)");
    return NNFAC_ERR_UNSUPPORTED;
  }
  const Side* cs = &p->side[which == 0 ? 1 : 0];
  const Side* ps = &p->side[which];
  PeerG none;
  memset(&none, 0, sizeof(none));
  factor_finish_kernel<true, 64, false, 2, true><<<(unsigned)ceil_div64(len, 32), 256, 0, (cudaStream_t)stream>>>(
      p->partial, ps->cp.splits, p->r, p->r_pad, len, ps->cp.ld_partial, F_in, ld_in, 0, 0, none, den_partial, (float)floor_value,
      F_out, ld_out, cs->fh, cs->fl, cs->ld, p->rowp_h[which], p->rowp_l[which], nullptr, nullptr, (float)gamma);
  NNFAC_LAUNCH_CHECK(p->ctx);
  return NNFAC_OK;
}

}
```

nn-fac_b200/nn_fac/_lib.py:

```python
import ctypes
import os

import numpy as np
import torch

_HERE = os.path.dirname(os.path.abspath(__file__))
LIB_PATH = os.environ.get("NNFAC_B200_LIB") or os.path.join(os.path.dirname(_HERE), "lib", "libnnfac_b200.so")

F32, F64 = 0, 1
ERR_UNSUPPORTED = -3
HALS_NORMALIZE, HALS_NONZERO, HALS_NO_TC = 1, 2, 4

_c = ctypes
_P, _I64, _INT, _DBL, _U32 = _c.c_void_p, _c.c_int64, _c.c_int, _c.c_double, _c.c_uint

SIGNATURES = {
    "nnfac_abi_version": [],
    "nnfac_last_error": [],
    "nnfac_ctx_create": [_INT, _c.POINTER(_P)],
    "nnfac_ctx_destroy": [_P],
    "nnfac_ctx_sm_count": [_P],
    "nnfac_ctx_launch_count": [_P],
    "nnfac_ctx_board_export": [_P, _P],
    "nnfac_ctx_board_attach": [_P, _INT, _INT, _P],
    "nnfac_ctx_collective": [_P, _INT, _P],
    "nnfac_ctx_sweep_variant": [_P, _INT],
    "nnfac_xchg_create": [_P, _I64, _I64, _c.POINTER(_P)],
    "nnfac_xchg_export": [_P, _P],
    "nnfac_xchg_attach": [_P, _INT, _INT, _P],
    "nnfac_xchg_destroy": [_P],
    "nnfac_xchg_ptr": [_P, _INT],
    "nnfac_xchg_post": [_P, _INT, _P],
    "nnfac_xchg_post_tail": [_P, _P, _INT, _I64, _I64, _P],
    "nnfac_xchg_pull_tail": [_P, _INT, _P, _I64, _INT, _I64, _I64, _INT, _P],
    "nnfac_nmf_plan_set_factor_pulled": [_P, _INT, _P, _I64, _I64, _P, _I64, _P],
    "nnfac_hals_nnls": [_P, _INT, _P, _I64, _P, _I64, _P, _I64, _INT, _I64, _INT, _DBL, _DBL, _U32, _P, _P],
    "nnfac_hals_solve_f32": [_P, _P, _I64, _P, _I64, _P, _I64, _P, _I64, _INT, _I64, _INT, _DBL, _DBL, _P, _P],
    "nnfac_hals_solve_slabs_f32": [_P, _P, _I64, _INT, _I64, _INT, _P, _P, _I64, _P, _I64, _P, _I64, _INT, _I64, _INT, _DBL, _DBL, _P, _P],
    "nnfac_xchg_inbox_mu_apply": [_P, _I64, _INT, _I64, _I64, _I64, _P, _I64, _INT, _I64, _I64, _DBL, _I64, _P],
    "nnfac_nmf_plan_set_push": [_P, _P, _I64, _I64, _c.POINTER(_INT), _c.POINTER(_I64)],
    "nnfac_reduce_slabs_f32": [_P, _P, _I64, _INT, _INT, _INT, _I64, _P, _I64, _P],
    "nnfac_gemm_strided": [_P, _INT, _P, _I64, _I64, _P, _I64, _I64, _I64, _I64, _P, _I64, _I64, _I64, _I64,
                           _I64, _I64, _I64, _I64, _I64, _P],
    "nnfac_gram": [_P, _INT, _P, _I64, _P, _I64, _INT, _I64, _P],
    "nnfac_mu_terms": [_P, _INT, _DBL, _P, _P, _P, _P, _I64, _P],
    "nnfac_mu_apply": [_P, _INT, _P, _P, _P, _P, _P, _INT, _I64, _I64, _DBL, _DBL, _P],
    "nnfac_beta_divergence": [_P, _INT, _DBL, _P, _P, _I64, _P, _P],
    "nnfac_sq_diff": [_P, _INT, _P, _P, _I64, _P, _P],
    "nnfac_dot": [_P, _INT, _P, _P, _I64, _P, _P],
    "nnfac_row_sums": [_P, _INT, _P, _I64, _I64, _I64, _P, _P],
    "nnfac_norm1": [_P, _INT, _P, _I64, _I64, _I64, _P, _P],
    "nnfac_transpose": [_P, _INT, _P, _I64, _P, _I64, _I64, _I64, _P],
    "nnfac_khatri_rao": [_P, _INT, _P, _P, _I64, _P, _I64, _I64, _P],
    "nnfac_hadamard": [_P, _INT, _P, _P, _P, _I64, _P],
    "nnfac_axpby": [_P, _INT, _P, _DBL, _P, _DBL, _P, _I64, _P],
    "nnfac_normalize_rows": [_P, _INT, _P, _I64, _I64, _I64, _P],
    "nnfac_core_pg_step": [_P, _INT, _P, _P, _P, _I64, _DBL, _DBL, _DBL, _P, _P],
    "nnfac_core_pg_step_dev": [_P, _INT, _P, _P, _P, _I64, _DBL, _P, _P],
    "nnfac_core_pg_step3": [_P, _INT, _P, _P, _P, _P, _P, _INT, _INT, _INT, _P, _DBL, _DBL, _INT, _DBL, _P, _P],
    "nnfac_philox_uniform": [_P, _P, _I64, _I64, _I64, _I64, _I64, _c.c_uint64, _U32, _DBL, _INT, _P],
    "nnfac_nmf_plan_create": [_P, _I64, _I64, _INT, _c.POINTER(_P)],
    "nnfac_nmf_plan_bytes": [_P, _I64, _I64, _INT, _c.POINTER(_c.c_size_t)],
    "nnfac_nmf_plan_create_in": [_P, _I64, _I64, _INT, _P, _c.c_size_t, _P, _c.POINTER(_P)],
    "nnfac_nmf_plan_bytes_sided": [_P, _I64, _I64, _INT, _INT, _c.POINTER(_c.c_size_t)],
    "nnfac_nmf_plan_create_sided": [_P, _I64, _I64, _INT, _INT, _P, _c.c_size_t, _P, _c.POINTER(_P)],
    "nnfac_nmf_plan_bytes_planes": [_P, _I64, _I64, _INT, _INT, _INT, _c.POINTER(_c.c_size_t)],
    "nnfac_nmf_plan_create_planes": [_P, _I64, _I64, _INT, _INT, _INT, _P, _c.c_size_t, _P, _c.POINTER(_P)],
    "nnfac_nmf_plan_view_bytes": [_P, _P, _I64, _I64, _I64, _INT, _c.POINTER(_c.c_size_t)],
    "nnfac_nmf_plan_create_view": [_P, _P, _I64, _I64, _I64, _INT, _P, _c.c_size_t, _P, _c.POINTER(_P)],
    "nnfac_nmf_plan_destroy": [_P],
    "nnfac_nmf_plan_load_x": [_P, _P, _I64, _P],
    "nnfac_nmf_plan_load_x_rows": [_P, _P, _I64, _I64, _I64, _P],
    "nnfac_nmf_plan_load_x_done": [_P, _P],
    "nnfac_nmf_plan_f32_bytes": [_P, _c.POINTER(_c.c_size_t)],
    "nnfac_nmf_plan_enable_f32": [_P, _P, _c.c_size_t, _P],
    "nnfac_nmf_plan_cross": [_P, _INT, _P, _I64, _P, _I64, _P],
    "nnfac_nmf_plan_set_factor": [_P, _INT, _P, _I64, _P],
    "nnfac_nmf_plan_set_factor_gathered": [_P, _INT, _P, _I64, _P, _I64, _P],
    "nnfac_nmf_plan_reduce": [_P, _INT, _P, _I64, _P],
    "nnfac_nmf_plan_reduce_chunked": [_P, _INT, _P, _I64, _INT, _P, _I64, _INT, _P],
    "nnfac_nmf_plan_set_krao": [_P, _P, _I64, _I64, _P, _I64, _I64, _P],
    "nnfac_nmf_plan_set_krao_rows": [_P, _P, _I64, _I64, _P, _I64, _I64, _P],
    "nnfac_nmf_plan_hals_solve": [_P, _INT, _P, _I64, _P, _I64, _P, _I64, _P, _I64, _INT, _DBL, _DBL, _P, _P],
    "nnfac_nmf_plan_fused": [_P, _INT, _INT, _INT, _P, _I64, _P, _P],
    "nnfac_nmf_plan_mu_finish": [_P, _INT, _P, _I64, _P, _DBL, _P, _I64, _P],
    "nnfac_nmf_plan_fused_beta_bytes": [_P, _c.POINTER(_c.c_size_t)],
    "nnfac_nmf_plan_fused_beta": [_P, _INT, _DBL, _INT, _P, _P, _P],
    "nnfac_nmf_plan_mu_finish_beta": [_P, _INT, _P, _I64, _P, _DBL, _DBL, _P, _I64, _P],
    "nnfac_nmf_plan_info": [_P, _INT, _c.POINTER(_INT), _c.POINTER(_INT), _c.POINTER(_INT), _c.POINTER(_INT),
                            _c.POINTER(_INT)],
}
_RESTYPES = {"nnfac_last_error": _c.c_char_p, "nnfac_ctx_launch_count": _I64, "nnfac_xchg_ptr": _P}

_lib = None
_ctxs = {}


class NnfacError(RuntimeError):
    """A call into libnnfac_b200 failed (status < 0); the message comes from nnfac_last_error()."""


def load_library():
    global _lib
    if _lib is not None:
        return _lib
    if not os.path.exists(LIB_PATH):
        raise ImportError(f"{LIB_PATH} is missing: build it with `bash nn-fac_b200/build.sh` "
                          "(python -c 'import __graft_entry__ as g; g.build()'). There is no CPU fallback.")
    lib = ctypes.CDLL(LIB_PATH)
    for name, args in SIGNATURES.items():
        fn = getattr(lib, name)
        fn.argtypes = args
        fn.restype = _RESTYPES.get(name, _INT)
    if lib.nnfac_abi_version() != 1:
        raise ImportError("libnnfac_b200.so ABI version mismatch")
    _lib = lib
    return lib


def check(status):
    if status != 0:
        raise NnfacError(f"nnfac status {status}: {load_library().nnfac_last_error().decode()}")


_cuda_ok = None


def device_index(device=None):
    global _cuda_ok
    if _cuda_ok is None:
        if not torch.cuda.is_available():
            raise NnfacError("nn_fac (B200 build) needs a CUDA device; there is no CPU fallback")
        _cuda_ok = True
    if device is None:
        return torch.cuda.current_device()
    if isinstance(device, torch.device):
        return device.index or 0
    return torch.device(device).index or 0


def ctx(device=None):
    idx = device_index(device)
    if idx not in _ctxs:
        handle = _P()
        check(load_library().nnfac_ctx_create(idx, ctypes.byref(handle)))
        _ctxs[idx] = handle
    return _ctxs[idx]


def launch_count(device=None):
    return int(load_library().nnfac_ctx_launch_count(ctx(device)))


_raw_stream = getattr(torch._C, "_cuda_getCurrentRawStream", None)


def stream_ptr():
    if _raw_stream is not None:
        return _P(_raw_stream(torch.cuda.current_device()))
    return _P(torch.cuda.current_stream().cuda_stream)


def code_of(dtype):
    if dtype == torch.float32:
        return F32
    if dtype == torch.float64:
        return F64
    raise NnfacError(f"unsupported dtype {dtype}")


def ptr(t):
    return _P(t.data_ptr()) if t is not None else _P(None)


def to_device(x, dtype, device=None):
    dev = torch.device("cuda", device_index(device))
    if isinstance(x, torch.Tensor):
        return x.to(device=dev, dtype=dtype).contiguous()
    arr = np.ascontiguousarray(np.asarray(x))
    return torch.from_numpy(arr).to(device=dev, dtype=dtype)


def resolve_dtype(*arrays):
    from . import config
    if config.precision == "fp32":
        return torch.float32
    if config.precision in ("fp64", "fp32x3"):
        return torch.float64
    for a in arrays:
        if a is None:
            continue
        dt = a.dtype
        if dt in (torch.float32, np.float32) or str(dt) == "float32":
            continue
        return torch.float64
    return torch.float32


def as_output(x):
    from . import config
    if config.precision != "fp32x3":
        return x
    if isinstance(x, torch.Tensor):
        return x if x.dtype == torch.float32 else x.to(torch.float32)
    x = np.asarray(x)
    return x if x.dtype == np.float32 else x.astype(np.float32)


def working_dtype(numel, *arrays):
    from . import config
    if config.precision == "fp32x3":
        return torch.float64, torch.float32
    dt = resolve_dtype(*arrays)
    if dt == torch.float32 and config.precision == "auto" and int(numel) <= config.small_problem_elements:
        return torch.float64, torch.float32
    return dt, dt
```

Before: 775.5.

## Fold cost finish into fused kernel via last-block reduction; fetch D1 early

Replaces the separate single-thread cost-sum kernel launch with a last-arriving-block reduction inside the fused kernel, using an atomic arrive counter stored past the cost partials. For MU with deferred cost, the epilogue warps also issue the next D1 TMEM fetch and reload X during the deferred log-cost loop, and release the X stage afterwards. This is meant to overlap latency and remove a launch. The cost is holding ring stages longer, plus extra global atomics and fences. It also adds optional clock-based profiling macros and a standalone cost-finish entry point.

```diff
diff --git a/include/nnfac_b200.h b/include/nnfac_b200.h
--- a/include/nnfac_b200.h
+++ b/include/nnfac_b200.h
@@ -161,6 +161,9 @@
 int nnfac_nmf_plan_fused_beta_bytes(const nnfac_nmf_plan* plan, size_t* bytes);
 int nnfac_nmf_plan_fused_beta(nnfac_nmf_plan* plan, int side, double beta, int want_cost, float* den_partial, double* cost_out,
                               void* stream);
+
+int nnfac_nmf_plan_cost_parts_finish(nnfac_nmf_plan* plan, int side, int kl, double* cost_out, void* stream);
+
 int nnfac_nmf_plan_mu_finish_beta(nnfac_nmf_plan* plan, int which, const float* F_in, int64_t ld_in, const float* den_partial,
                                   double gamma, double floor_value, float* F_out, int64_t ld_out, void* stream);
 int nnfac_nmf_plan_info(const nnfac_nmf_plan* plan, int which, int* splits, int* stages_per_unit,
diff --git a/nn-fac_b200/csrc/tc_common.cuh b/nn-fac_b200/csrc/tc_common.cuh
--- a/nn-fac_b200/csrc/tc_common.cuh
+++ b/nn-fac_b200/csrc/tc_common.cuh
@@ -55,6 +55,14 @@
   }
 }
 
+__device__ __forceinline__ uint32_t mbar_wait_polls(uint64_t* bar, uint32_t parity) {
+  uint32_t fails = 0;
+  uint64_t t0 = 0;
+  while (!mbar_try_wait(bar, parity))
+    if ((++fails & 4095u) == 0u) mbar_wait_timeout_check(t0);
+  return fails;
+}
+
 __device__ __forceinline__ void fence_proxy_async_smem() {
   asm volatile("fence.proxy.async.shared::cta;" ::: "memory");
 }
diff --git a/nn-fac_b200/csrc/tc_fused.cu b/nn-fac_b200/csrc/tc_fused.cu
--- a/nn-fac_b200/csrc/tc_fused.cu
+++ b/nn-fac_b200/csrc/tc_fused.cu
@@ -22,7 +22,49 @@
 #ifndef FUSED_DEFER_COST
 #define FUSED_DEFER_COST 1
 #endif
+#ifndef FUSED_EARLY_FETCH
+#define FUSED_EARLY_FETCH 1
+#endif
+#ifndef FUSED_EARLY_AT
+#define FUSED_EARLY_AT 0
+#endif
 constexpr int DRAIN = 2;
+
+#ifdef FUSED_PROF
+__device__ unsigned long long g_fused_prof[4][32];
+#define FPROF_INIT                                                    \
+  uint32_t prof_acc = 0, prof_t = (uint32_t)clock();                  \
+  auto prof_add = [&](int s_, uint32_t v_) { if (lane == s_) prof_acc += v_; };                            \
+  auto prof_flush = [&](int role_) { atomicAdd(&g_fused_prof[role_][lane], (unsigned long long)prof_acc); };
+#define FPROF_INIT1                                                   \
+  uint32_t prof_arr[32];                                              \
+  for (int s_ = 0; s_ < 32; ++s_) prof_arr[s_] = 0;                   \
+  uint32_t prof_t = (uint32_t)clock();                                \
+  auto prof_add = [&](int s_, uint32_t v_) { prof_arr[s_] += v_; };                                         \
+  auto prof_flush = [&](int role_) { for (int s_ = 0; s_ < 32; ++s_) atomicAdd(&g_fused_prof[role_][s_], (unsigned long long)prof_arr[s_]); };
+#define FPROF_MARK(s)                                                 \
+  do {                                                                \
+    const uint32_t n_ = (uint32_t)clock();                            \
+    prof_add(s, n_ - prof_t);                                         \
+    prof_t = n_;                                                      \
+  } while (0)
+#define FPROF_WAIT(s, bar, par)                                       \
+  do {                                                                \
+    FPROF_MARK(15);                                                   \
+    const uint32_t f_ = tc::mbar_wait_polls(bar, par);                \
+    FPROF_MARK(s);                                                    \
+    prof_add(16 + (s), f_);                                           \
+  } while (0)
+#define FPROF_STAGE() prof_add(31, 1u)
+#define FPROF_FLUSH(role) do { FPROF_MARK(15); prof_flush(role); } while (0)
+#else
+#define FPROF_INIT
+#define FPROF_INIT1
+#define FPROF_MARK(s) do { } while (0)
+#define FPROF_WAIT(s, bar, par) tc::mbar_wait(bar, par)
+#define FPROF_STAGE() do { } while (0)
+#define FPROF_FLUSH(role) do { } while (0)
+#endif
 
 template <int RK, int PLANES = 2, bool XF32 = false>
 struct Cfg {
@@ -47,6 +89,10 @@
   float* push[NNFAC_MAX_PEERS];
   int64_t push_chunk;
   int push_src;
+  double* cost_out;
+  const double* sums;
+  unsigned* arrive;
+  int cost_kl;
 };
 
 constexpr int NHC = 11;
@@ -110,6 +156,34 @@
   }
   return kb * h;
 }
+__device__ __forceinline__ double kl_cost_total(const double* part, int n, const double* sums) {
+  double s = 0.0, sk = 0.0;
+  for (int i = 0; i < n; ++i) { s += part[i]; sk += part[512 + i]; }
+  constexpr double a0 = 6.05e-8, a1 = -4.0e-8;
+  s = __fma_rn(-a0, sums[0], __dmul_rn(1.0 - a1, s));
+  return __dadd_rn(__fma_rn(0.6931471805599453, s, -sums[0]), sk);
+}
+__device__ __forceinline__ double cost_parts_total(const double* part, int n) {
+  double s = 0.0;
+  for (int i = 0; i < n; ++i) s += part[i];
+  return s;
+}
+__device__ __noinline__ void finish_cost(const double* part, const double* sums, int kl, double* out, unsigned* arrive,
+                                        double* scratch, uint32_t gen, int lane) {
+  __threadfence();
+  const int n = (int)gridDim.x;
+  for (int i = lane; i < n; i += 32) {
+    scratch[i] = __ldcg(part + i);
+    scratch[512 + i] = __ldcg(part + 512 + i);
+  }
+  __syncwarp();
+  if (lane == 0) {
+    *out = kl ? kl_cost_total(scratch, n, sums) : cost_parts_total(scratch, n);
+    *reinterpret_cast<volatile unsigned*>(arrive + 1) = gen + (unsigned)n;
+  }
+  __syncwarp();
+}
+
 __device__ __forceinline__ float bf_lo(uint32_t w) { return __uint_as_float(w << 16); }
 __device__ __forceinline__ float bf_hi(uint32_t w) { return __uint_as_float(w & 0xffff0000u); }
 
@@ -176,11 +250,12 @@
 
   if (warp == 0 && lane == 0) {
     int stage = 0; uint32_t phase = 0, a1_phase = 0;
+    FPROF_INIT1
     for (int u = blockIdx.x; u < p.num_units; u += gridDim.x) {
       const int tile = p.split_major ? u % p.tiles : u / p.splits, split = p.split_major ? u / p.tiles : u % p.splits;
       const int row0 = tile * TILE_ROWS, k0 = split * S * BK;
       if (RK == 64) {
-        tc::mbar_wait(a1_empty, a1_phase ^ 1);
+        FPROF_WAIT(0, a1_empty, a1_phase ^ 1);
         a1_phase ^= 1;
         tc::mbar_arrive_expect_tx(a1_full, A1_BYTES);
         tc::tma_load_2d_hint(a1, &map_a1h, a1_full, 0, row0, tc::kEvictLast);
@@ -188,7 +263,7 @@
         if (PLANES == 3) tc::tma_load_2d_hint(a1 + 2 * X_BYTES, &map_a1m, a1_full, 0, row0, tc::kEvictLast);
       }
       for (int ks = 0; ks < S; ++ks) {
-        tc::mbar_wait(&empty[stage], phase ^ 1);
+        FPROF_WAIT(1, &empty[stage], phase ^ 1);
         uint8_t* st = ring + (size_t)stage * STAGE_BYTES;
         tc::mbar_arrive_expect_tx(&full[stage], STAGE_BYTES);
         const int c = k0 + ks * BK;
@@ -201,21 +276,25 @@
           tc::tma_load_2d_hint(st + XB + FK_BYTES + kr * 8192, &map_fkl, &full[stage], kr * 64, c, tc::kEvictLast);
           if (PLANES == 3) tc::tma_load_2d_hint(st + XB + 2 * FK_BYTES + kr * 8192, &map_fkm, &full[stage], kr * 64, c, tc::kEvictLast);
         }
+        FPROF_MARK(2);
+        FPROF_STAGE();
         if (++stage == FSTAGES) { stage = 0; phase ^= 1; }
       }
     }
+    FPROF_FLUSH(0);
   } else if (warp == 1) {
     const uint32_t idesc1 = tc::umma_idesc_bf16(TILE_ROWS, 64);
     const int ksteps = p.r_pad / UMMA_K;
     int st1 = 0; uint32_t ph1 = 0;
     int b1 = 0; uint32_t b1_phase = 0;
     uint32_t a1_phase = 0;
+    FPROF_INIT
     for (int u = blockIdx.x; u < p.num_units; u += gridDim.x) {
-      tc::mbar_wait(BETA ? a1_full : a1t_ready, a1_phase);
+      FPROF_WAIT(0, BETA ? a1_full : a1t_ready, a1_phase);
       a1_phase ^= 1;
       for (int i = 0; i < S; ++i) {
-        tc::mbar_wait(&full[st1], ph1);
-        tc::mbar_wait(&d1_empty[b1], b1_phase ^ 1);
+        FPROF_WAIT(1, &full[st1], ph1);
+        FPROF_WAIT(2, &d1_empty[b1], b1_phase ^ 1);
         tc::tcgen05_fence_after();
         if (tc::elect_one()) {
           const uint32_t sb = tc::smem_u32(ring + (size_t)st1 * STAGE_BYTES);
@@ -264,22 +343,26 @@
           if (i == S - 1) tc::umma_commit(BETA ? a1_empty : a1t_free);
         }
         __syncwarp();
+        FPROF_MARK(3);
+        FPROF_STAGE();
         if (++b1 == ND1) { b1 = 0; b1_phase ^= 1; }
         if (++st1 == FSTAGES) { st1 = 0; ph1 ^= 1; }
       }
     }
+    FPROF_FLUSH(1);
   } else if (warp == 3) {
     const uint32_t idesc2 = tc::umma_idesc_bf16(TILE_ROWS, p.r_pad) | (1u << 16);
     int qb = 0; uint32_t qb_phase = 0;
     int st2 = 0; uint32_t ph2 = 0;
     int b2 = 0; uint32_t b2_phase = 0;
+    FPROF_INIT
     for (int u = blockIdx.x; u < p.num_units; u += gridDim.x) {
       for (int j = 0; j < S; ++j) {
         const bool chain_start = (j % DRAIN_P) == 0;
         const bool chain_end = ((j + 1) % DRAIN_P) == 0 || j == S - 1;
-        tc::mbar_wait(&full[st2], ph2);
-        if (MODE == MODE_MU || BETA) tc::mbar_wait(&q_ready[qb], qb_phase);
-        if (chain_start) tc::mbar_wait(&d2_empty[b2], b2_phase ^ 1);
+        FPROF_WAIT(0, &full[st2], ph2);
+        if (MODE == MODE_MU || BETA) FPROF_WAIT(1, &q_ready[qb], qb_phase);
+        if (chain_start) FPROF_WAIT(2, &d2_empty[b2], b2_phase ^ 1);
         tc::tcgen05_fence_after();
         if (tc::elect_one()) {
           const uint32_t sb = tc::smem_u32(ring + (size_t)st2 * STAGE_BYTES);
@@ -349,11 +432,14 @@
           if (chain_end) tc::umma_commit(&d2_full[b2]);
         }
         __syncwarp();
+        FPROF_MARK(3);
+        FPROF_STAGE();
         if (MODE == MODE_MU || BETA) { if (++qb == NQ) { qb = 0; qb_phase ^= 1; } }
         if (chain_end) { if (++b2 == 2) { b2 = 0; b2_phase ^= 1; } }
         if (++st2 == FSTAGES) { st2 = 0; ph2 ^= 1; }
       }
     }
+    FPROF_FLUSH(2);
   } else if (warp >= 4) {
     const int q = warp & 3, part = (warp - 4) >> 2;
     const int row = q * 32 + lane;
@@ -364,6 +450,7 @@
     int qb = 0; uint32_t qb_phase = 0;
     uint32_t a1_phase = 0;
     double cost = 0.0, costk = 0.0;
+    FPROF_INIT
     for (int u = blockIdx.x; u < p.num_units; u += gridDim.x) {
       const int tile = p.split_major ? u % p.tiles : u / p.splits, split = p.split_major ? u / p.tiles : u % p.splits;
       float sum[CWD], sumd[BETA ? CWD : 1];
@@ -373,8 +460,8 @@
 #pragma unroll
         for (int j = 0; j < CWD; ++j) sumd[BETA ? j : 0] = 0.f;
       } else if (RK == 64) {
-        tc::mbar_wait(a1_full, a1_phase);
-        tc::mbar_wait(a1t_free, a1_phase ^ 1);
+        FPROF_WAIT(0, a1_full, a1_phase);
+        FPROF_WAIT(0, a1t_free, a1_phase ^ 1);
         a1_phase ^= 1;
         tc::tcgen05_fence_after();
 #pragma unroll
@@ -392,6 +479,7 @@
         tc::tcgen05_fence_before();
         __syncwarp();
         if (lane == 0) { tc::mbar_arrive(a1t_ready); tc::mbar_arrive(a1_empty); }
+        FPROF_MARK(1);
       } else {
         const int64_t grow = (int64_t)tile * TILE_ROWS + row;
         uint32_t w[2][16];
@@ -404,7 +492,7 @@
             w[pl][4 * c] = v4.x; w[pl][4 * c + 1] = v4.y; w[pl][4 * c + 2] = v4.z; w[pl][4 * c + 3] = v4.w;
           }
         }
-        tc::mbar_wait(a1t_free, a1_phase ^ 1);
+        FPROF_WAIT(0, a1t_free, a1_phase ^ 1);
         a1_phase ^= 1;
         tc::tcgen05_fence_after();
         tc::tmem_st16(A1T + lane_base + (RK / 8) * part, w[0]);
@@ -413,9 +501,10 @@
         tc::tcgen05_fence_before();
         __syncwarp();
         if (lane == 0) tc::mbar_arrive(a1t_ready);
+        FPROF_MARK(1);
       }
       auto drain_chain = [&]() {
-        tc::mbar_wait(&d2_full[b2], b2_phase);
+        FPROF_WAIT(10, &d2_full[b2], b2_phase);
         tc::tcgen05_fence_after();
 #pragma unroll
         for (int c0 = 0; c0 < CWD; c0 += 16) {
@@ -437,6 +526,7 @@
         __syncwarp();
         if (lane == 0) tc::mbar_arrive(&d2_empty[b2]);
         if (++b2 == 2) { b2 = 0; b2_phase ^= 1; }
+        FPROF_MARK(11);
       };
       int drained = 0;
       float2 acc2 = make_float2(0.f, 0.f), acck2 = make_float2(0.f, 0.f);
@@ -444,7 +534,7 @@
       uint32_t kn[CW];
       int bf = b1; uint32_t bf_phase = b1_phase;
       auto fetch_d1 = [&]() {
-        tc::mbar_wait(&d1_full[bf], bf_phase);
+        FPROF_WAIT(2, &d1_full[bf], bf_phase);
         tc::tcgen05_fence_after();
         tc::tmem_ld16(D1 + (uint32_t)bf * 64 + lane_base + CW * part, kn);
         if (++bf == ND1) { bf = 0; bf_phase ^= 1; }
@@ -452,9 +542,12 @@
 #if FUSED_PREFETCH
       fetch_d1();
 #endif
+      constexpr bool EARLY = FUSED_EARLY_FETCH && !FUSED_PREFETCH && FUSED_DEFER_COST && FUSED_PACKED && MODE == MODE_MU && COST &&
+                             PLANES == 2;
+      constexpr int EARLY_AT = FUSED_EARLY_AT;
       for (int i = 0; i < S; ++i) {
 #if !FUSED_PREFETCH
-        fetch_d1();
+        if (!EARLY || i == 0) fetch_d1();
 #endif
         tc::tmem_ld_wait16(kn);
         uint32_t kk[CW];
@@ -464,19 +557,18 @@
         __syncwarp();
         if (lane == 0) tc::mbar_arrive(&d1_empty[b1]);
         if (++b1 == ND1) { b1 = 0; b1_phase ^= 1; }
+        FPROF_MARK(3);
 #if FUSED_PREFETCH
         if (i + 1 < S) fetch_d1();
 #endif
-        tc::mbar_wait(&full[st], ph);
+        FPROF_WAIT(4, &full[st], ph);
         uint8_t* xh = ring + (size_t)st * STAGE_BYTES;
         uint8_t* xl = xh + X_BYTES;
         uint32_t qhw[4 * NCHK], qlw[4 * NCHK];
         constexpr bool DEFER = FUSED_DEFER_COST && FUSED_PACKED && MODE == MODE_MU && COST;
         float2 xs[DEFER ? 4 * NCHK : 1], qs[DEFER ? 4 * NCHK : 1];
         uint32_t dhw[BETA ? 4 * NCHK : 1], dlw[BETA ? 4 * NCHK : 1];
-#pragma unroll
-        for (int cc = 0; cc < NCHK; ++cc) {
-          float2 xv[4];
+        auto load_x = [&](int cc, float2 (&xv)[4]) {
           if (XF32) {
             const uint8_t* xb = xh + (size_t)(part >> 1) * X_BYTES + (uint32_t)row * 128u;
 #pragma unroll
@@ -508,6 +600,11 @@
 #endif
             }
           }
+        };
+#pragma unroll
+        for (int cc = 0; cc < NCHK; ++cc) {
+          float2 xv[4];
+          load_x(cc, xv);
           if constexpr (BETA) {
 #pragma unroll
             for (int w = 0; w < 4; ++w) {
@@ -602,11 +699,15 @@
           }
         };
         if (!DEFER) flush_cost();
-        __syncwarp();
-        if (lane == 0) tc::mbar_arrive(&empty[st]);
-        if (++st == FSTAGES) { st = 0; ph ^= 1; }
+        FPROF_MARK(5);
+        auto release_x = [&]() {
+          __syncwarp();
+          if (lane == 0) tc::mbar_arrive(&empty[st]);
+          if (++st == FSTAGES) { st = 0; ph ^= 1; }
+        };
+        if (!EARLY) release_x();
         if (MODE == MODE_MU) {
-          tc::mbar_wait(&q_free[qb], qb_phase ^ 1);
+          FPROF_WAIT(7, &q_free[qb], qb_phase ^ 1);
           tc::tcgen05_fence_after();
           const uint32_t qa = QT + (uint32_t)qb * 64 + lane_base + (CW / 2) * part;
           tc::tmem_st8(qa, qhw);
@@ -616,22 +717,28 @@
           __syncwarp();
           if (lane == 0) tc::mbar_arrive(&q_ready[qb]);
           if (++qb == NQ) { qb = 0; qb_phase ^= 1; }
+          FPROF_MARK(8);
           if (DEFER) {
+            float2 xr[4];
 #pragma unroll
             for (int e = 0; e < 4 * NCHK; ++e) {
+              if (EARLY && e == EARLY_AT && i + 1 < S) fetch_d1();
+              if (EARLY && (e & 3) == 0) load_x(e >> 2, xr);
               if constexpr (PLANES == 3) {
                 const float2 k2 = make_float2(__uint_as_float(kk[2 * e]), __uint_as_float(kk[2 * e + 1]));
                 acc2 = __ffma2_rn(k2, make_float2(kl_g(qs[DEFER ? e : 0].x), kl_g(qs[DEFER ? e : 0].y)), acc2);
               } else {
                 const float2 qt = __fadd2_rn(qs[DEFER ? e : 0], tiny2);
-                acc2 = __ffma2_rn(xs[DEFER ? e : 0], make_float2(lg2_approx(qt.x), lg2_approx(qt.y)), acc2);
+                acc2 = __ffma2_rn(EARLY ? xr[e & 3] : xs[DEFER ? e : 0], make_float2(lg2_approx(qt.x), lg2_approx(qt.y)), acc2);
               }
             }
+            if (EARLY) release_x();
             flush_cost();
+            FPROF_MARK(9);
           }
         }
         if constexpr (BETA) {
-          tc::mbar_wait(&q_free[0], qb_phase ^ 1);
+          FPROF_WAIT(7, &q_free[0], qb_phase ^ 1);
           tc::tcgen05_fence_after();
           const uint32_t qa = QT + lane_base + (CW / 2) * part;
           tc::tmem_st8(qa, qhw);
@@ -643,8 +750,10 @@
           __syncwarp();
           if (lane == 0) tc::mbar_arrive(&q_ready[0]);
           qb_phase ^= 1;
+          FPROF_MARK(8);
         }
         if (DRAIN_P == 2 ? (i >= 3 && (i & 1)) : i >= 2) { drain_chain(); ++drained; }
+        FPROF_STAGE();
       }
       for (; drained < (S + DRAIN_P - 1) / DRAIN_P; ++drained) drain_chain();
       if (p.push_chunk > 0) {
@@ -666,19 +775,32 @@
             if (CWD * part + j < p.r_pad) outd[(int64_t)j * p.ld_partial] = sumd[BETA ? j : 0];
         }
       }
+      FPROF_MARK(12);
     }
     if (COST) {
       cost = warp_sum(cost);
       if (MODE == MODE_MU) costk = warp_sum(costk);
       if (lane == 0) { cost_sh[warp - 4] = cost; cost_sh[NWT + warp - 4] = costk; }
       asm volatile("bar.sync 1, %0;" ::"n"(32 * NWT) : "memory");
-      if (warp == 4 && lane == 0) {
-        double t = 0.0, tk = 0.0;
-        for (int w = 0; w < NWT; ++w) { t += cost_sh[w]; tk += cost_sh[NWT + w]; }
-        p.cost_part[blockIdx.x] = t;
-        p.cost_part[512 + blockIdx.x] = tk;
+      if (warp == 4) {
+        uint32_t gen = 0, last = 0;
+        if (lane == 0) {
+          double t = 0.0, tk = 0.0;
+          for (int w = 0; w < NWT; ++w) { t += cost_sh[w]; tk += cost_sh[NWT + w]; }
+          p.cost_part[blockIdx.x] = t;
+          p.cost_part[512 + blockIdx.x] = tk;
+          if (p.cost_out) {
+            gen = *reinterpret_cast<volatile unsigned*>(p.arrive + 1);
+            __threadfence();
+            last = atomicAdd(p.arrive, 1u) - gen == gridDim.x - 1;
+          }
+        }
+        if (p.cost_out && __shfl_sync(0xffffffffu, last, 0))
+          finish_cost(p.cost_part, p.sums, p.cost_kl, p.cost_out, p.arrive, reinterpret_cast<double*>(ring), gen, lane);
       }
+      FPROF_MARK(13);
     }
+    FPROF_FLUSH(3);
   }
   tc::tcgen05_fence_before();
   __syncthreads();
@@ -794,22 +916,8 @@
   }
 }
 
-__global__ void sum_cost_parts_kernel(const double* part, int n, double* out) {
-  if (threadIdx.x == 0) {
-    double s = 0.0;
-    for (int i = 0; i < n; ++i) s += part[i];
-    out[0] = s;
-  }
-}
-
-__global__ void kl_cost_finish_kernel(const double* part, int n, const double* sums, double* out) {
-  if (threadIdx.x == 0) {
-    double s = 0.0, sk = 0.0;
-    for (int i = 0; i < n; ++i) { s += part[i]; sk += part[512 + i]; }
-    constexpr double a0 = 6.05e-8, a1 = -4.0e-8;
-    s = (1.0 - a1) * s - a0 * sums[0];
-    out[0] = 0.6931471805599453 * s - sums[0] + sk;
-  }
+__global__ void cost_finish_kernel(const double* part, int n, const double* sums, int kl, double* out) {
+  if (threadIdx.x == 0) out[0] = kl ? kl_cost_total(part, n, sums) : cost_parts_total(part, n);
 }
 
 template <int PLANES>
@@ -874,10 +982,22 @@
   fp.a1h = p->rowp_h[side]; fp.a1l = p->rowp_l[side]; fp.R = s->R;
   fp.push_chunk = 0; fp.push_src = 0;
   for (int q = 0; q < NNFAC_MAX_PEERS; ++q) fp.push[q] = nullptr;
+  fp.cost_out = nullptr; fp.sums = p->sums; fp.cost_kl = 0;
+  fp.arrive = reinterpret_cast<unsigned*>(p->cost_part + 2047);
   return fp;
 }
 
 extern "C" {
+
+#ifdef FUSED_PROF
+int nnfac_fused_prof_read(unsigned long long* out) {
+  NNFAC_CUDA(cudaDeviceSynchronize());
+  NNFAC_CUDA(cudaMemcpyFromSymbol(out, g_fused_prof, sizeof(g_fused_prof)));
+  static const unsigned long long zero[4][32] = {};
+  NNFAC_CUDA(cudaMemcpyToSymbol(g_fused_prof, zero, sizeof(zero)));
+  return NNFAC_OK;
+}
+#endif
 
 int nnfac_nmf_plan_f32_bytes(const nnfac_nmf_plan* p, size_t* bytes) {
   NNFAC_ARG(p && bytes, "nnfac_nmf_plan_f32_bytes: NULL argument");
@@ -1042,6 +1162,10 @@
   NNFAC_ARG(!out || ld_out >= s->R, "nnfac_nmf_plan_fused: leading dimension too small");
   cudaStream_t st = (cudaStream_t)stream;
   FusedParams fp = fused_params(p, side, mode == 0 || want_cost);
+  if (fp.want_cost && cost_out) {
+    fp.cost_out = cost_out;
+    fp.cost_kl = mode == 1 && p->planes == 2;
+  }
   BetaParams bp;
   memset(&bp, 0, sizeof(bp));
   if (side == 0 && !out && p->push_chunk > 0) {
@@ -1085,13 +1209,13 @@
     nnfac_reduce_partials(p->partial, fp.splits, p->r, p->r_pad, s->R, fp.ld_partial, out, ld_out, p->ctx->sm_count, st);
     NNFAC_LAUNCH_CHECK(p->ctx);
   }
-  if (cost_out && fp.want_cost) {
-    if (mode == 0 || p->planes == 3)
-      sum_cost_parts_kernel<<<1, 32, 0, st>>>(p->cost_part, s->grid, cost_out);
-    else
-      kl_cost_finish_kernel<<<1, 32, 0, st>>>(p->cost_part, s->grid, p->sums, cost_out);
-    NNFAC_LAUNCH_CHECK(p->ctx);
-  }
+  return NNFAC_OK;
+}
+
+int nnfac_nmf_plan_cost_parts_finish(nnfac_nmf_plan* p, int side, int kl, double* cost_out, void* stream) {
+  NNFAC_ARG(p && cost_out && (side == 0 || side == 1), "nnfac_nmf_plan_cost_parts_finish: bad argument");
+  cost_finish_kernel<<<1, 32, 0, (cudaStream_t)stream>>>(p->cost_part, p->side[side].grid, p->sums, kl, cost_out);
+  NNFAC_LAUNCH_CHECK(p->ctx);
   return NNFAC_OK;
 }
 
@@ -1113,7 +1237,8 @@
   if (p->push_chunk > 0) { nnfac_set_error("nnfac_nmf_plan_fused_beta: not available with the push exchange (nnfac_nmf_plan_set_push)"); return NNFAC_ERR_UNSUPPORTED; }
   Side* s = &p->side[side];
   cudaStream_t st = (cudaStream_t)stream;
-  const FusedParams fp = fused_params(p, side, want_cost != 0);
+  FusedParams fp = fused_params(p, side, want_cost != 0);
+  if (fp.want_cost) fp.cost_out = cost_out;
   BetaParams bp;
   memset(&bp, 0, sizeof(bp));
   bp.den = den_partial;
@@ -1143,10 +1268,6 @@
 #undef NNFAC_LAUNCH_BETA_X
 #undef NNFAC_LAUNCH_BETA
   NNFAC_LAUNCH_CHECK(p->ctx);
-  if (cost_out && fp.want_cost) {
-    sum_cost_parts_kernel<<<1, 32, 0, st>>>(p->cost_part, s->grid, cost_out);
-    NNFAC_LAUNCH_CHECK(p->ctx);
-  }
   return NNFAC_OK;
 }
 
diff --git a/nn-fac_b200/nn_fac/_lib.py b/nn-fac_b200/nn_fac/_lib.py
--- a/nn-fac_b200/nn_fac/_lib.py
+++ b/nn-fac_b200/nn_fac/_lib.py
@@ -86,6 +86,7 @@
     "nnfac_nmf_plan_mu_finish": [_P, _INT, _P, _I64, _P, _DBL, _P, _I64, _P],
     "nnfac_nmf_plan_fused_beta_bytes": [_P, _c.POINTER(_c.c_size_t)],
     "nnfac_nmf_plan_fused_beta": [_P, _INT, _DBL, _INT, _P, _P, _P],
+    "nnfac_nmf_plan_cost_parts_finish": [_P, _INT, _INT, _P, _P],
     "nnfac_nmf_plan_mu_finish_beta": [_P, _INT, _P, _I64, _P, _DBL, _DBL, _P, _I64, _P],
     "nnfac_nmf_plan_info": [_P, _INT, _c.POINTER(_INT), _c.POINTER(_INT), _c.POINTER(_INT), _c.POINTER(_INT),
                             _c.POINTER(_INT)],
```

After: 752.7 (median of 6 runs). 2.9% lower.
